# joshuagryphon/plastid

Measured on AMD Instinct MI355X. Metric: mapped_reads_per_sec, higher is better.
Workload: dtype int64; 1 GPU; C2: 100 M synthetic single-end reads, FivePrimeMapFactory(offset=12), 20 k yeast-scale transcripts; records=100000000, chains=20000, segments=21031, output_positions=33373947, tiles=5922

## Files before the change

### include/plastid_counts.h

```cpp
#ifndef PLASTID_COUNTS_H
#define PLASTID_COUNTS_H

#include <stdint.h>

#ifdef __cplusplus
extern "C" {
#endif

#define PC_ABI_VERSION 23

typedef struct pc_engine pc_engine;
typedef struct pc_plan pc_plan;

#define PC_OK 0
#define PC_ERR_ARG (-1)
#define PC_ERR_HIP (-2)
#define PC_ERR_NOMEM (-3)
#define PC_ERR_UNSORTED (-4)
#define PC_ERR_STATE (-5)

#define PC_MAP_FIVE 0
#define PC_MAP_THREE 1
#define PC_MAP_CENTER 2
#define PC_MAP_VAR5 3
#define PC_MAP_STRAT5 4

#define PC_STRAND_UNDEF 0
#define PC_STRAND_FWD 1
#define PC_STRAND_REV 2
#define PC_STRAND_UNS 3
#define PC_STRAND_NOFILTER 0x10

#define PC_FLAG_REVERSE 0x01
#define PC_FLAG_EXCLUDED 0x80

#define PC_OUT_INT64 0
#define PC_OUT_FLOAT64 1

#define PC_OFFSET_TABLE_LEN 10000
#define PC_MAX_ALIGNED_LEN 65535

const char *pc_last_error(void);
int pc_abi_version(void);
int pc_device_count(void);

int pc_create(int device, pc_engine **out);
int pc_destroy(pc_engine *e);
int pc_release_cached_memory(int device);
int pc_host_alloc(pc_engine *e, uint64_t bytes, void **out);
int pc_host_free(pc_engine *e, void *p);
int pc_reload_knobs(pc_engine *e);

int pc_clear_alignments(pc_engine *e);
int pc_add_alignment_file(pc_engine *e, int64_t n, int32_t ntid, const int32_t *tid,
                          const int32_t *pos, const uint16_t *alen, const uint8_t *flags,
                          const uint8_t *nblk, int64_t nrun, const int32_t *blk_start,
                          const int32_t *blk_len);
int pc_add_alignment_file_wide(pc_engine *e, int64_t n, int32_t ntid, const int32_t *tid,
                               const int32_t *pos, const uint16_t *alen, const uint8_t *flags,
                               const uint8_t *nblk, int64_t nrun, const int32_t *blk_start,
                               const int32_t *blk_len, int64_t n_wide, const int64_t *wide_idx,
                               const int32_t *wide_alen, const int32_t *wide_nblk);
int pc_update_flags(pc_engine *e, int file, int64_t n, const uint8_t *flags);
int pc_num_files(pc_engine *e);
int64_t pc_num_records(pc_engine *e, int file);
int64_t pc_stream_entries(pc_engine *e, int file);
int64_t pc_canonical_entries(pc_engine *e, int file);
int64_t pc_dense_cells(pc_engine *e, int file);
#define PC_DENSE_PATH_NONE 0
#define PC_DENSE_PATH_ITEMS 1
#define PC_DENSE_PATH_CHUNKS 2
int pc_dense_path(pc_engine *e);
int pc_read_records(pc_engine *e, int file, int64_t n, const int64_t *idx, int32_t *tid, int32_t *pos, int32_t *alen, uint8_t *reverse,
                    int32_t *nblk, uint16_t *flag16, uint8_t *mapq);
int pc_read_record_runs(pc_engine *e, int file, int64_t n, const int64_t *idx, const int64_t *run_at, int64_t nruns, int32_t *start,
                        int32_t *len);

int pc_set_alignment_sam(pc_engine *e, int file, int64_t n, const uint16_t *flag, const uint8_t *mapq);
int pc_set_flag_filter(pc_engine *e, int enabled, uint32_t require, uint32_t exclude, int min_mapq);
int pc_set_alignment_nh(pc_engine *e, int file, int64_t n, const uint16_t *nh);
int pc_set_nh_filter(pc_engine *e, int max_nh);

int pc_set_mapping(pc_engine *e, int kind, int param, const int32_t *fw, const int32_t *rc,
                   int table_len, int min_len, int max_len);
int pc_set_size_filter(pc_engine *e, int enabled, int min_len, int max_len);
int pc_set_normalize(pc_engine *e, int enabled, double sum);
int pc_mapping_rows(pc_engine *e);

int pc_plan_create(pc_engine *e, int64_t nseg, const int32_t *tid, const int64_t *start,
                   const int64_t *end, const uint8_t *strand, const int64_t *out_off,
                   const int8_t *out_step, const int64_t *row_stride, int64_t out_elems, int rows,
                   pc_plan **out);
int pc_plan_destroy(pc_plan *p);
int pc_plan_coordinates(pc_engine *e, pc_plan *p, int64_t *host_out, int64_t out_elems);
int64_t pc_plan_positions(pc_plan *p);
int64_t pc_plan_tiles(pc_plan *p);
int pc_plan_table(pc_plan *p, int which, void *buf, int64_t cap_bytes, int64_t *bytes);

int pc_count(pc_engine *e, pc_plan *p, int out_dtype);
int pc_sync(pc_engine *e);
int pc_query_segment(pc_engine *e, int32_t tid, int64_t start, int64_t end, uint8_t strand, int reverse_out, int out_dtype,
                     void *host_out);
int pc_read_counts(pc_engine *e, pc_plan *p, void *host_out, int64_t out_elems);
void *pc_counts_device_ptr(pc_plan *p);
void *pc_stream(pc_engine *e);

int pc_rle(pc_engine *e, pc_plan *p, int64_t period, int64_t *n_runs);
int pc_read_rle(pc_engine *e, pc_plan *p, int64_t *starts, void *values, int64_t n_runs);

int pc_warn_flags(pc_engine *e, pc_plan *p, uint8_t *flags);
int pc_warn_details(pc_engine *e, pc_plan *p, uint8_t *flags, int32_t *last_len);

int pc_total(pc_engine *e, pc_plan *p, void *host_out8);
void *pc_total_device_ptr(pc_plan *p);

int pc_mapped_reads(pc_engine *e, int file, int64_t rec_lo, int64_t rec_hi, int32_t tid,
                    int64_t start, int64_t end, uint8_t strand, uint8_t *mask);

int pc_mapped_reads_batch(pc_engine *e, pc_plan *p, int64_t *offsets, int64_t *total);
int pc_read_mapped_reads(pc_engine *e, pc_plan *p, uint32_t *rec, int64_t total);

int pc_set_profiling(pc_engine *e, int level);
int pc_last_timing(pc_engine *e, double *ms, int n);
int64_t pc_last_algorithmic_bytes(pc_engine *e);
int pc_center_replay_steps(pc_engine *e, pc_plan *p, int64_t *steps, int64_t *waves);
int pc_center_row_fill(pc_engine *e, pc_plan *p, int64_t *row_entries, int64_t *row_slots);
int pc_stream_probe(pc_engine *e, int64_t bytes, int iters, double *read_gbps, double *write_gbps);

typedef struct pc_bam pc_bam;
int pc_bam_open(pc_engine *e, const void *image, int64_t size, const char *name , pc_bam **out);
int pc_bam_counts(pc_bam *b, int64_t *counts8);
int pc_bam_timing(pc_bam *b, double *ms4);
int pc_bam_nref(pc_bam *b);
const char *pc_bam_ref_name(pc_bam *b, int i);
int32_t pc_bam_ref_length(pc_bam *b, int i);
int pc_bam_read(pc_bam *b, int32_t *tid, int32_t *pos, uint16_t *alen, uint8_t *flags, uint8_t *nblk, int32_t *blk_start,
                int32_t *blk_len, int64_t *wide_idx, int32_t *wide_alen, int32_t *wide_nblk);
int pc_bam_read_sam(pc_bam *b, uint16_t *flag, uint8_t *mapq, int32_t *lseq);
int pc_bam_read_nh(pc_bam *b, uint16_t *nh);
int pc_bam_close(pc_bam *b);
int pc_add_alignment_bam(pc_engine *e, const void *image, int64_t size, const char *name, int64_t *mapped);
int pc_bam_open_path(pc_engine *e, const char *path, pc_bam **out);
int pc_add_alignment_bam_path(pc_engine *e, const char *path, int64_t *mapped);
int pc_bam_open_span(pc_engine *e, const char *path, uint64_t voff_begin, uint64_t voff_end, int nreg, const int32_t *tid,
                     const int64_t *beg, const int64_t *end, pc_bam **out);
int pc_add_alignment_bam_span(pc_engine *e, const char *path, uint64_t voff_begin, uint64_t voff_end, int nreg, const int32_t *tid,
                              const int64_t *beg, const int64_t *end, int64_t *mapped);
int pc_bam_open_chunks(pc_engine *e, const char *path, int nchunk, const uint64_t *voff_beg, const uint64_t *voff_end, int nreg,
                       const int32_t *tid, const int64_t *beg, const int64_t *end, pc_bam **out);
int pc_add_alignment_bam_chunks(pc_engine *e, const char *path, int nchunk, const uint64_t *voff_beg, const uint64_t *voff_end,
                                int nreg, const int32_t *tid, const int64_t *beg, const int64_t *end, int64_t *mapped);
int pc_bam_stats(pc_bam *b, int64_t *out4);
#define PC_BAM_SORT 1u
int pc_bam_open_flags(pc_engine *e, const void *image, int64_t size, const char *name, uint32_t flags, pc_bam **out);
int pc_bam_open_path_flags(pc_engine *e, const char *path, uint32_t flags, pc_bam **out);
int pc_add_alignment_bam_flags(pc_engine *e, const void *image, int64_t size, const char *name, uint32_t flags, int64_t *mapped);
int pc_add_alignment_bam_path_flags(pc_engine *e, const char *path, uint32_t flags, int64_t *mapped);
int pc_bam_sort_stats(pc_bam *b, int64_t *out4, double *ms);
int pc_bam_read_file_order(pc_bam *b, int64_t *rec_no);

int pc_sam_open_path_flags(pc_engine *e, const char *path, uint32_t flags, pc_bam **out);
int pc_sam_open_flags(pc_engine *e, const void *image, int64_t size, const char *name, uint32_t flags, pc_bam **out);
int pc_add_alignment_sam_path_flags(pc_engine *e, const char *path, uint32_t flags, int64_t *mapped);

typedef struct pc_bam_index pc_bam_index;
int pc_bam_index_build(pc_engine *e, const char *path, pc_bam_index **out);
int pc_bam_index_finish(int n_ref, int64_t n_runs, const int32_t *run_tid, const uint32_t *run_bin, const uint64_t *run_beg,
                        const uint64_t *run_end, const int64_t *lin_start, const uint64_t *linear, const uint64_t *ref_beg,
                        const uint64_t *ref_end, const int64_t *ref_mapped, const int64_t *ref_unmapped, int64_t n_no_coor,
                        pc_bam_index **out);
int pc_bam_index_build_csi(pc_engine *e, const char *path, int min_shift, pc_bam_index **out);
int pc_bam_index_finish_csi(int min_shift, int n_lvls, int n_ref, int64_t n_runs, const int32_t *run_tid, const uint32_t *run_bin,
                            const uint64_t *run_beg, const uint64_t *run_end, const uint64_t *run_loff, const uint64_t *ref_beg,
                            const uint64_t *ref_end, const int64_t *ref_mapped, const int64_t *ref_unmapped, int64_t n_no_coor,
                            pc_bam_index **out);
int pc_bam_index_bytes(pc_bam_index *idx, void *buf, int64_t cap, int64_t *bytes);
int pc_bam_index_stats(pc_bam_index *idx, int64_t *out8);
int pc_bam_index_timing(pc_bam_index *idx, double *ms8);
int pc_bam_index_close(pc_bam_index *idx);

typedef struct pc_track pc_track;
int pc_track_create(pc_engine *e, int nstrands, int64_t min_chr_size, pc_track **out);
int pc_track_destroy(pc_track *t);
int pc_track_declare(pc_track *t, const char *name, int64_t length);
int pc_track_add_text(pc_track *t, const void *image, int64_t size, const char *name, int strand_slot);
int pc_track_add_path(pc_track *t, const char *path, int strand_slot);
int pc_track_num_contigs(pc_track *t);
const char *pc_track_contig_name(pc_track *t, int i);
int64_t pc_track_contig_length(pc_track *t, int i);
int64_t pc_track_contig_extent(pc_track *t, int i, int strand_slot);
int pc_track_gather(pc_track *t, int64_t nseg, const int32_t *contig, const int32_t *strand_slot, const int64_t *start, const int64_t *end,
                    const int64_t *out_off, const int8_t *out_step, int64_t out_elems, int normalize, double *host_out);
int pc_track_sum(pc_track *t, double *sum);
int pc_track_stats(pc_track *t, int64_t *out6);
int pc_track_timing(pc_track *t, double *ms5);

int pc_track_set(pc_track *t, const char *contig, int strand_slot, int64_t nseg, const int64_t *start, const int64_t *end, const int64_t *val_off,
                 const int8_t *val_step, const double *values, int64_t nvalues, double scalar);
int pc_track_combine(pc_track *a, pc_track *b, double scalar, int op, int mode_all, int64_t length_pad, int nstrands_out, const int32_t *slot_a,
                     const int32_t *slot_b, pc_track **out);
int pc_track_equal(pc_track *a, pc_track *b, int64_t npair, const int32_t *contig_a, const int32_t *slot_a, const int32_t *contig_b, const int32_t *slot_b,
                   double tol, int *equal);
int pc_track_nonzero_count(pc_track *t, int64_t *counts);
int pc_track_nonzero_read(pc_track *t, int64_t *out, int64_t total);
int pc_track_export(pc_track *t, int kind, int strand_slot, int64_t *bytes);
int pc_track_export_read(pc_track *t, void *dst, int64_t bytes);
int pc_track_export_stats(pc_track *t, int64_t *out4);
int pc_track_export_timing(pc_track *t, double *ms6);
int pc_track_export_geometry(int *out2);

int pc_counts_export_batches(int64_t n, const int64_t *len, int64_t budget, int32_t *batch_of, int *nbatch);
int pc_counts_export(pc_engine *e, pc_plan *p, int kind, int64_t period, int nrange, const char *const *names, const int64_t *elem_off,
                     const int64_t *len, int64_t *bytes);
int pc_counts_export_read(pc_engine *e, void *dst, int64_t bytes);
int pc_counts_export_stats(pc_engine *e, int64_t *out4);
int pc_counts_export_timing(pc_engine *e, double *ms6);
int pc_track_set_counts(pc_track *t, const char *contig, int strand_slot, int64_t start, pc_plan *p, int64_t elem_off, int64_t n);

int pc_bigwig_info(const char *path, const void *image, int64_t size, int64_t *out5, int max_contigs, char *names, int64_t names_bytes, int64_t *sizes);
int pc_bigwig_blocks(const char *path, const void *image, int64_t size, int64_t nblocks, int64_t *off, int64_t *bytes);
// ... 40 lines not shown
```

### plastid_amd/_lib.py

```python
import ctypes
import os

from .exceptions import EngineError

HERE = os.path.dirname(os.path.abspath(__file__))
LIB_PATH = os.environ.get("PLASTID_AMD_LIB") or os.path.join(HERE, "libplastid_counts.so")

PC_OK = 0
PC_ERR_ARG = -1
PC_ERR_HIP = -2
PC_ERR_NOMEM = -3
PC_ERR_UNSORTED = -4
PC_ERR_STATE = -5

MAP_FIVE, MAP_THREE, MAP_CENTER, MAP_VAR5, MAP_STRAT5 = 0, 1, 2, 3, 4
STRAND_UNDEF, STRAND_FWD, STRAND_REV, STRAND_UNS = 0, 1, 2, 3
STRAND_NOFILTER = 0x10
OUT_INT64, OUT_FLOAT64 = 0, 1
OFFSET_TABLE_LEN = 10000

_vp, _i64, _i32, _int = ctypes.c_void_p, ctypes.c_int64, ctypes.c_int32, ctypes.c_int
_pp = ctypes.POINTER(ctypes.c_void_p)
SIGNATURES = {
    "pc_last_error": (ctypes.c_char_p, []),
    "pc_abi_version": (_int, []),
    "pc_device_count": (_int, []),
    "pc_create": (_int, [_int, _pp]),
    "pc_destroy": (_int, [_vp]),
    "pc_reload_knobs": (_int, [_vp]),
    "pc_clear_alignments": (_int, [_vp]),
    "pc_add_alignment_file": (_int, [_vp, _i64, _i32, _vp, _vp, _vp, _vp, _vp, _i64, _vp, _vp]),
    "pc_add_alignment_file_wide": (_int, [_vp, _i64, _i32, _vp, _vp, _vp, _vp, _vp, _i64, _vp, _vp, _i64, _vp, _vp, _vp]),
    "pc_update_flags": (_int, [_vp, _int, _i64, _vp]),
    "pc_set_alignment_sam": (_int, [_vp, _int, _i64, _vp, _vp]),
    "pc_set_flag_filter": (_int, [_vp, _int, ctypes.c_uint32, ctypes.c_uint32, _int]),
    "pc_set_alignment_nh": (_int, [_vp, _int, _i64, _vp]),
    "pc_set_nh_filter": (_int, [_vp, _int]),
    "pc_num_files": (_int, [_vp]),
    "pc_num_records": (_i64, [_vp, _int]),
    "pc_stream_entries": (_i64, [_vp, _int]),
    "pc_canonical_entries": (_i64, [_vp, _int]),
    "pc_dense_cells": (_i64, [_vp, _int]),
    "pc_dense_path": (_int, [_vp]),
    "pc_read_records": (_int, [_vp, _int, _i64] + [_vp] * 8),
    "pc_read_record_runs": (_int, [_vp, _int, _i64, _vp, _vp, _i64, _vp, _vp]),
    "pc_set_mapping": (_int, [_vp, _int, _int, _vp, _vp, _int, _int, _int]),
    "pc_set_size_filter": (_int, [_vp, _int, _int, _int]),
    "pc_set_normalize": (_int, [_vp, _int, ctypes.c_double]),
    "pc_mapping_rows": (_int, [_vp]),
    "pc_plan_create": (_int, [_vp, _i64, _vp, _vp, _vp, _vp, _vp, _vp, _vp, _i64, _int, _pp]),
    "pc_plan_destroy": (_int, [_vp]),
    "pc_plan_positions": (_i64, [_vp]),
    "pc_plan_coordinates": (_int, [_vp, _vp, _vp, _i64]),
    "pc_plan_tiles": (_i64, [_vp]),
    "pc_plan_table": (_int, [_vp, _int, _vp, _i64, ctypes.POINTER(_i64)]),
    "pc_count": (_int, [_vp, _vp, _int]),
    "pc_sync": (_int, [_vp]),
    "pc_query_segment": (_int, [_vp, _i32, _i64, _i64, ctypes.c_uint8, _int, _int, _vp]),
    "pc_release_cached_memory": (_int, [_int]),
    "pc_host_alloc": (_int, [_vp, ctypes.c_uint64, ctypes.POINTER(ctypes.c_void_p)]),
    "pc_host_free": (_int, [_vp, _vp]),
    "pc_read_counts": (_int, [_vp, _vp, _vp, _i64]),
    "pc_counts_device_ptr": (_vp, [_vp]),
    "pc_stream": (_vp, [_vp]),
    "pc_rle": (_int, [_vp, _vp, _i64, ctypes.POINTER(_i64)]),
    "pc_read_rle": (_int, [_vp, _vp, _vp, _vp, _i64]),
    "pc_warn_flags": (_int, [_vp, _vp, _vp]),
    "pc_warn_details": (_int, [_vp, _vp, _vp, _vp]),
    "pc_total": (_int, [_vp, _vp, _vp]),
    "pc_total_device_ptr": (_vp, [_vp]),
    "pc_mapped_reads": (_int, [_vp, _int, _i64, _i64, _i32, _i64, _i64, ctypes.c_uint8, _vp]),
    "pc_mapped_reads_batch": (_int, [_vp, _vp, _vp, ctypes.POINTER(_i64)]),
    "pc_read_mapped_reads": (_int, [_vp, _vp, _vp, _i64]),
    "pc_set_profiling": (_int, [_vp, _int]),
    "pc_last_timing": (_int, [_vp, _vp, _int]),
    "pc_last_algorithmic_bytes": (_i64, [_vp]),
    "pc_center_replay_steps": (_int, [_vp, _vp, ctypes.POINTER(_i64), ctypes.POINTER(_i64)]),
    "pc_center_row_fill": (_int, [_vp, _vp, ctypes.POINTER(_i64), ctypes.POINTER(_i64)]),
    "pc_stream_probe": (_int, [_vp, _i64, _int, _vp, _vp]),
    "pc_bam_open": (_int, [_vp, _vp, _i64, ctypes.c_char_p, _pp]),
    "pc_bam_counts": (_int, [_vp, _vp]),
    "pc_bam_timing": (_int, [_vp, _vp]),
    "pc_bam_nref": (_int, [_vp]),
    "pc_bam_ref_name": (ctypes.c_char_p, [_vp, _int]),
    "pc_bam_ref_length": (_i32, [_vp, _int]),
    "pc_bam_read": (_int, [_vp] * 11),
    "pc_bam_read_sam": (_int, [_vp, _vp, _vp, _vp]),
    "pc_bam_read_nh": (_int, [_vp, _vp]),
    "pc_bam_close": (_int, [_vp]),
    "pc_add_alignment_bam": (_int, [_vp, _vp, _i64, ctypes.c_char_p, ctypes.POINTER(_i64)]),
    "pc_bam_open_path": (_int, [_vp, ctypes.c_char_p, _pp]),
    "pc_add_alignment_bam_path": (_int, [_vp, ctypes.c_char_p, ctypes.POINTER(_i64)]),
    "pc_bam_open_span": (_int, [_vp, ctypes.c_char_p, ctypes.c_uint64, ctypes.c_uint64, _int, _vp, _vp, _vp, _pp]),
    "pc_add_alignment_bam_span": (_int, [_vp, ctypes.c_char_p, ctypes.c_uint64, ctypes.c_uint64, _int, _vp, _vp, _vp, ctypes.POINTER(_i64)]),
    "pc_bam_open_chunks": (_int, [_vp, ctypes.c_char_p, _int, _vp, _vp, _int, _vp, _vp, _vp, _pp]),
    "pc_add_alignment_bam_chunks": (_int, [_vp, ctypes.c_char_p, _int, _vp, _vp, _int, _vp, _vp, _vp, ctypes.POINTER(_i64)]),
    "pc_bam_stats": (_int, [_vp, _vp]),
    "pc_bam_open_flags": (_int, [_vp, _vp, _i64, ctypes.c_char_p, ctypes.c_uint32, _pp]),
    "pc_bam_open_path_flags": (_int, [_vp, ctypes.c_char_p, ctypes.c_uint32, _pp]),
    "pc_add_alignment_bam_flags": (_int, [_vp, _vp, _i64, ctypes.c_char_p, ctypes.c_uint32, ctypes.POINTER(_i64)]),
    "pc_add_alignment_bam_path_flags": (_int, [_vp, ctypes.c_char_p, ctypes.c_uint32, ctypes.POINTER(_i64)]),
    "pc_bam_sort_stats": (_int, [_vp, _vp, _vp]),
    "pc_bam_read_file_order": (_int, [_vp, _vp]),
    "pc_sam_open_path_flags": (_int, [_vp, ctypes.c_char_p, ctypes.c_uint32, _pp]),
    "pc_sam_open_flags": (_int, [_vp, _vp, _i64, ctypes.c_char_p, ctypes.c_uint32, _pp]),
    "pc_add_alignment_sam_path_flags": (_int, [_vp, ctypes.c_char_p, ctypes.c_uint32, ctypes.POINTER(_i64)]),
    "pc_bam_index_build": (_int, [_vp, ctypes.c_char_p, _pp]),
    "pc_bam_index_finish": (_int, [_int, _i64] + [_vp] * 10 + [_i64, _pp]),
    "pc_bam_index_build_csi": (_int, [_vp, ctypes.c_char_p, _int, _pp]),
    "pc_bam_index_finish_csi": (_int, [_int, _int, _int, _i64] + [_vp] * 9 + [_i64, _pp]),
    "pc_bam_index_bytes": (_int, [_vp, _vp, _i64, ctypes.POINTER(_i64)]),
    "pc_bam_index_stats": (_int, [_vp, _vp]),
    "pc_bam_index_timing": (_int, [_vp, _vp]),
    "pc_bam_index_close": (_int, [_vp]),
    "pc_track_create": (_int, [_vp, _int, _i64, _pp]),
    "pc_track_destroy": (_int, [_vp]),
    "pc_track_declare": (_int, [_vp, ctypes.c_char_p, _i64]),
    "pc_track_add_text": (_int, [_vp, _vp, _i64, ctypes.c_char_p, _int]),
    "pc_track_add_path": (_int, [_vp, ctypes.c_char_p, _int]),
    "pc_track_num_contigs": (_int, [_vp]),
    "pc_track_contig_name": (ctypes.c_char_p, [_vp, _int]),
    "pc_track_contig_length": (_i64, [_vp, _int]),
    "pc_track_contig_extent": (_i64, [_vp, _int, _int]),
    "pc_track_gather": (_int, [_vp, _i64, _vp, _vp, _vp, _vp, _vp, _vp, _i64, _int, _vp]),
    "pc_track_sum": (_int, [_vp, ctypes.POINTER(ctypes.c_double)]),
    "pc_track_stats": (_int, [_vp, _vp]),
    "pc_track_timing": (_int, [_vp, _vp]),
    "pc_track_set": (_int, [_vp, ctypes.c_char_p, _int, _i64, _vp, _vp, _vp, _vp, _vp, _i64, ctypes.c_double]),
    "pc_track_combine": (_int, [_vp, _vp, ctypes.c_double, _int, _int, _i64, _int, _vp, _vp, _pp]),
    "pc_track_equal": (_int, [_vp, _vp, _i64, _vp, _vp, _vp, _vp, ctypes.c_double, ctypes.POINTER(_int)]),
    "pc_track_nonzero_count": (_int, [_vp, _vp]),
    "pc_track_nonzero_read": (_int, [_vp, _vp, _i64]),
    "pc_track_export": (_int, [_vp, _int, _int, ctypes.POINTER(_i64)]),
    "pc_track_export_read": (_int, [_vp, _vp, _i64]),
    "pc_track_export_stats": (_int, [_vp, _vp]),
    "pc_track_export_timing": (_int, [_vp, _vp]),
    "pc_track_export_geometry": (_int, [_vp]),
    "pc_counts_export_batches": (_int, [_i64, _vp, _i64, _vp, ctypes.POINTER(_int)]),
    "pc_counts_export": (_int, [_vp, _vp, _int, _i64, _int, _vp, _vp, _vp, ctypes.POINTER(_i64)]),
    "pc_counts_export_read": (_int, [_vp, _vp, _i64]),
    "pc_counts_export_stats": (_int, [_vp, _vp]),
    "pc_counts_export_timing": (_int, [_vp, _vp]),
    "pc_track_set_counts": (_int, [_vp, ctypes.c_char_p, _int, _i64, _vp, _i64, _i64]),
    "pc_bigwig_info": (_int, [ctypes.c_char_p, _vp, _i64, _vp, _int, _vp, _i64, _vp]),
    "pc_bigwig_blocks": (_int, [ctypes.c_char_p, _vp, _i64, _i64, _vp, _vp]),
    "pc_inflate_zlib": (_int, [_vp, _vp, _i64, _vp, _vp, _i64, _vp, _vp, _vp]),
    "pc_deflate_zlib": (_int, [_vp, _vp, _i64, _vp, _vp, _vp, _i64, _vp, _vp]),
    "pc_deflate_zlib_mode": (_int, [_vp, _vp, _i64, _vp, _vp, _vp, _i64, _vp, _vp, _int]),
    "pc_huffman_lengths": (_int, [_vp, _vp, _i64, _int, _vp]),
    "pc_track_export_bigwig": (_int, [_vp, _int, _i64, _i64, _int, _vp]),
    "pc_track_export_bigwig_zoom": (_int, [_vp, _int, _i64, _i64, _int, _i64, _vp]),
    "pc_track_export_bigwig_read": (_int, [_vp, _vp, _i64]),
    "pc_track_set_length": (_int, [_vp, ctypes.c_char_p, _i64]),
    "pc_track_bigwig_export_stats": (_int, [_vp, _vp]),
    "pc_track_bigwig_export_block_types": (_int, [_vp, _vp]),
    "pc_track_bigwig_export_timing": (_int, [_vp, _vp]),
    "pc_track_bigwig_export_zoom_stats": (_int, [_vp, _vp, _vp]),
    "pc_track_bigwig_export_zoom_timing": (_int, [_vp, _vp]),
    "pc_track_add_bigwig": (_int, [_vp, _vp, _i64, ctypes.c_char_p, _int]),
    "pc_track_add_bigwig_path": (_int, [_vp, ctypes.c_char_p, _int]),
    "pc_track_bigwig_stats": (_int, [_vp, _vp]),
    "pc_track_bigwig_timing": (_int, [_vp, _vp]),
    "pc_track_gather_sum": (_int, [_int, _vp, _i64, _vp, _vp, _vp, _vp, _vp, _vp, _i64, _int, ctypes.c_double, _vp]),
    "pc_track_sum_ranges": (_int, [_vp, _i64, _vp, _vp, _vp, _vp, ctypes.POINTER(ctypes.c_double)]),
    "pc_bigwig_summary_open": (_int, [_vp, _vp, _i64, ctypes.c_char_p, _pp]),
    "pc_bigwig_summary_open_path": (_int, [_vp, ctypes.c_char_p, _pp]),
    "pc_bigwig_summary_close": (_int, [_vp]),
    "pc_bigwig_summary_query": (_int, [_vp, _i64, _vp, _vp, _vp, _i64, _vp]),
    "pc_bigwig_summary_stats": (_int, [_vp, _vp, _int, _vp]),
    "pc_bigwig_summary_timing": (_int, [_vp, _vp]),
}

_lib = None


PC_BAM_SORT = 1

ABI_VERSION = 23


def load():
    global _lib
    if _lib is not None:
        return _lib
    if not os.path.exists(LIB_PATH):
        raise EngineError(
            "HIP counting library %s is missing. Build it with "
            "`python -m plastid_amd.build` (needs hipcc, gfx950). "
            "There is no CPU fallback." % LIB_PATH)
    try:
        lib = ctypes.CDLL(LIB_PATH)
    except OSError as e:
        raise EngineError("cannot load %s: %s" % (LIB_PATH, e))
    try:
        lib.pc_abi_version.restype = _int
        have = lib.pc_abi_version()
    except AttributeError:
        have = None
    if have != ABI_VERSION:
        raise EngineError("%s implements ABI revision %s, this package needs %d: rebuild it with `python -m plastid_amd.build --force`"
                          % (LIB_PATH, have, ABI_VERSION))
    for name, (res, args) in SIGNATURES.items():
        fn = getattr(lib, name)
        fn.restype = res
        fn.argtypes = args
    _lib = lib
    return lib


def last_error():
    msg = load().pc_last_error()
    return msg.decode("utf-8", "replace") if msg else ""


def check(rc, what=""):
    if rc == PC_OK:
        return
    msg = last_error() or what
    if rc in (PC_ERR_ARG, PC_ERR_UNSORTED):
        raise ValueError(msg)
    if rc == PC_ERR_NOMEM:
        raise MemoryError(msg)
    raise EngineError(msg)
```

### plastid_amd/csrc/dense_host.h

```cpp
#pragma once
#include <cstdint>

#if defined(__HIPCC__)
#define PCDENSE_HD __host__ __device__
#else
#define PCDENSE_HD
#endif

namespace pcdense {

constexpr int kItemLen = 2048;
constexpr uint32_t kEscape = 65535u;
constexpr int64_t kBytesPerCell = 2;
constexpr int64_t kBuildBlockCap = (int64_t)1 << 30;

PCDENSE_HD inline int64_t extent(int64_t declared, int64_t furthest_end) {
    const int64_t d = declared > 0 ? declared : 0, f = furthest_end > 0 ? furthest_end : 0;
    return d > f ? d : f;
}

inline int64_t layout(int ntid, const int64_t *ext, int64_t *cell_off) {
    int64_t at = 0;
    for (int t = 0; t < ntid; ++t)
        for (int s = 0; s < 2; ++s) { cell_off[2 * t + s] = at; at += ext[t]; }
    cell_off[2 * ntid] = at;
    return at;
}

struct PlanIn {
    int nfiles = 0;
    bool point_rule = false;
    int rows = 1;
    uint32_t modes = 0;
    bool has_sums = false;
    bool forbidden = false;
    int64_t cells = 0;
    int64_t stream_entries = 0;
};

inline bool plan_conditions(const PlanIn &p) {
    return !p.forbidden && p.nfiles == 1 && p.point_rule && p.rows == 1 && (p.modes & ~3u) == 0u && p.modes != 0u && !p.has_sums;
}
inline bool size_rule(int64_t cells, int64_t stream_entries) { return cells > 0 && cells * kBytesPerCell <= stream_entries * 4; }
inline bool build_fits(int64_t cells) { return cells * 8 <= kBuildBlockCap; }
inline bool eligible(const PlanIn &p) { return plan_conditions(p) && size_rule(p.cells, p.stream_entries) && build_fits(p.cells); }

struct SegIn {
    int64_t out_off = 0;
    int64_t len = 0;
    int64_t clip_lo = 0, clip_hi = 0;
    int64_t start = 0;
    int32_t step = 1;
    bool known = false;
    int64_t cell_base = 0;
    int64_t ext = 0;
};

struct Item {
    int64_t out_off;
    int64_t cell0;
    int32_t len, step, lo, hi;
};
static_assert(sizeof(Item) == 32, "Item is 32 bytes in HBM");

PCDENSE_HD inline int64_t items_of(int64_t len) { return len > 0 ? (len + kItemLen - 1) / kItemLen : 0; }

PCDENSE_HD inline Item cut_item(const SegIn &s, int64_t k) {
    const int64_t a = k * kItemLen;
    const int64_t n = s.len - a < kItemLen ? s.len - a : kItemLen;
    Item it;
    it.out_off = s.out_off + (int64_t)s.step * a;
    it.len = (int32_t)n; it.step = s.step; it.lo = 0; it.hi = 0; it.cell0 = -1;
    if (!s.known) return it;
    int64_t lo = s.clip_lo, hi = s.clip_hi;
    if (s.start + hi > s.ext) hi = s.ext - s.start;
    if (s.start + lo < 0) lo = -s.start;
    lo -= a; hi -= a;
    if (lo < 0) lo = 0;
    if (hi > n) hi = n;
    if (hi <= lo) return it;
    it.lo = (int32_t)lo; it.hi = (int32_t)hi;
    it.cell0 = s.cell_base + s.start + a;
    return it;
}

struct PairCut {
    int32_t head, pairs, tail;
};
PCDENSE_HD inline PairCut pair_cut(int64_t out_off, int32_t step, int32_t len) {
    PairCut c;
    c.head = (int32_t)((step > 0 ? out_off : out_off + 1) & 1);
    if (c.head > len) c.head = len;
    c.pairs = (len - c.head) >> 1;
    c.tail = (len - c.head) & 1;
    return c;
}
PCDENSE_HD inline int64_t pair_slot(int64_t out_off, int32_t step, const PairCut &c, int32_t p) {
    const int64_t i0 = c.head + 2 * (int64_t)p;
    return step > 0 ? out_off + i0 : out_off - i0 - 1;
}

#ifndef PC_DENSE_BATCH
#define PC_DENSE_BATCH 1
#endif
constexpr int kBatch = PC_DENSE_BATCH;
PCDENSE_HD inline int64_t batches_of(int64_t n_items) { return (n_items + kBatch - 1) / kBatch; }

#ifndef PC_DENSE_CHUNK
#define PC_DENSE_CHUNK 1024
#endif
constexpr int kChunk = PC_DENSE_CHUNK;
constexpr int kRow = 128;
constexpr int kInlineSpans = 7;
static_assert(kChunk % (4 * kRow) == 0 && kChunk / kRow <= 32, "a chunk is whole rows for four waves; its rows are the bits of a word");

struct Span {
    uint32_t ab, rr;
    uint32_t cell;
    int32_t dir;
    PCDENSE_HD uint32_t a() const { return ab & 0xffffu; }
    PCDENSE_HD uint32_t b() const { return ab >> 16; }
    PCDENSE_HD uint32_t ra() const { return rr & 0xffffu; }
    PCDENSE_HD uint32_t rb() const { return rr >> 16; }
};
static_assert(sizeof(Span) == 16, "Span is 16 bytes in HBM");
struct ChunkDesc {
    uint32_t n, ovf, pad[2];
    Span s[kInlineSpans];
};
static_assert(sizeof(ChunkDesc) == 128, "a descriptor is one line");

PCDENSE_HD inline int64_t chunks_of(int64_t out_elems) { return (out_elems + kChunk - 1) / kChunk; }
PCDENSE_HD inline int64_t seg_out_lo(int64_t out_off, int32_t step, int64_t len) { return step > 0 ? out_off : out_off - len + 1; }
PCDENSE_HD inline int64_t spans_of(int64_t out_lo, int64_t len) { return len > 0 ? (out_lo + len - 1) / kChunk - out_lo / kChunk + 1 : 0; }
inline bool spans_fit(int64_t nseg, int64_t covered) { return 2 * nseg + covered / kChunk < (int64_t)0xffffffffu; }

PCDENSE_HD inline Span cut_span(const SegIn &s, int64_t k) {
    const int64_t lo = seg_out_lo(s.out_off, s.step, s.len), base = (lo / kChunk + k) * kChunk;
    const int64_t a = lo > base ? lo : base, b = lo + s.len < base + kChunk ? lo + s.len : base + kChunk;
    int64_t plo = 0, phi = 0;
    if (s.known) {
        plo = s.clip_lo; phi = s.clip_hi;
        if (s.start + phi > s.ext) phi = s.ext - s.start;
        if (s.start + plo < 0) plo = -s.start;
        if (plo < 0) plo = 0;
        if (phi > s.len) phi = s.len;
    }
    int64_t ra = s.step > 0 ? s.out_off + plo : s.out_off - phi + 1, rb = s.step > 0 ? s.out_off + phi : s.out_off - plo + 1;
    if (ra < a) ra = a;
    if (rb > b) rb = b;
    if (phi <= plo || rb <= ra) ra = rb = a;
    Span sp;
    sp.ab = (uint32_t)(a - base) | (uint32_t)(b - base) << 16;
    sp.rr = (uint32_t)(ra - base) | (uint32_t)(rb - base) << 16;
    sp.dir = s.step > 0 ? 1 : -1;
    const int64_t pos = s.step > 0 ? a - s.out_off : s.out_off - a;
    sp.cell = (uint32_t)(s.cell_base + s.start + pos);
    return sp;
}
PCDENSE_HD inline bool span_reads(const Span &s, uint32_t e) { return e >= s.ra() && e < s.rb(); }
PCDENSE_HD inline uint32_t span_cell(const Span &s, uint32_t e) { return s.cell + (uint32_t)s.dir * (e - s.a()); }
PCDENSE_HD inline uint32_t span_rows(const Span &s) {
    const uint32_t ra = s.ra(), rb = s.rb();
    return ra < rb ? (2u << ((rb - 1u) / kRow)) - (1u << (ra / kRow)) : 0u;
}
PCDENSE_HD inline uint32_t span_base(const Span &s) { return s.cell - (uint32_t)s.dir * s.a(); }
PCDENSE_HD inline uint32_t base_cell(uint32_t base, bool up, uint32_t e) { return up ? base + e : base - e; }
PCDENSE_HD inline bool same_word(uint32_t x0, uint32_t x1) { return (x0 | 1u) == (x1 | 1u); }

PCDENSE_HD inline bool out_overlap(int64_t prev_lo, int64_t prev_len, int64_t lo) { return prev_lo + prev_len > lo; }
PCDENSE_HD inline bool first_of_chunk(int64_t lo, int64_t k, int64_t prev_end) {
    return k > 0 || lo % kChunk == 0 || prev_end < 0 || (prev_end - 1) / kChunk < lo / kChunk;
}
PCDENSE_HD inline ChunkDesc make_desc(const Span *spans, uint32_t first, uint32_t n) {
    ChunkDesc d;
    d.n = n; d.ovf = first + kInlineSpans; d.pad[0] = d.pad[1] = 0;
    for (int i = 0; i < kInlineSpans; ++i) {
        if ((uint32_t)i < n) d.s[i] = spans[first + i];
        else { d.s[i].ab = d.s[i].rr = 0; d.s[i].cell = 0; d.s[i].dir = 1; }
    }
    return d;
}

}
```

### plastid_amd/csrc/plastid_counts.hip

```cpp
#include "pc_kernels.hip.h"
#include "plan_kernels.hip.h"
#include "stage_kernels.hip.h"
#include "dense_kernels.hip.h"

#include <hipcub/hipcub.hpp>

#include <algorithm>
#include <atomic>
#include <cstdarg>
#include <cstdio>
#include <cstdlib>
#include <cstring>
#include <string>
#include <chrono>
#include <future>
#include <functional>
#include <condition_variable>
#include <map>
#include <mutex>
#include <unistd.h>
#include <mutex>
#include <sched.h>
#include <sys/mman.h>
#include <sys/stat.h>
// ... 228 lines not shown
            if (hipGetDevice(&dev_now) == hipSuccess) BigReservoir::get().free_all(dev_now);
            HIP_TRY(hipMalloc((void **)&p, n * sizeof(T)));
        }
        cap = n;
        return PC_OK;
    }
    int upload(const T *src, size_t n, hipStream_t s) {
        PC_TRY(reserve(n));
        if (n) HIP_TRY(hipMemcpyAsync(p, src, n * sizeof(T), hipMemcpyHostToDevice, s));
        return PC_OK;
    }
    int upload(const std::vector<T> &v, hipStream_t s) { return upload(v.data(), v.size(), s); }
    void swap(DevBuf &o) {
        std::swap(p, o.p); std::swap(cap, o.cap); std::swap(pool, o.pool); std::swap(pool_class, o.pool_class); std::swap(big_bytes, o.big_bytes);
    }
};

struct PinnedBuf {
    uint8_t *p = nullptr;
    size_t cap = 0;
    ~PinnedBuf() { if (p) (void)hipHostFree(p); }
    int reserve(size_t n) {
        if (n <= cap) return PC_OK;
        if (p) (void)hipHostFree(p);
        p = nullptr; cap = 0;
        const size_t want = std::max<size_t>(n + n / 2, 512 * 1024);
        HIP_TRY(hipHostMalloc((void **)&p, want, hipHostMallocDefault));
        cap = want;
        return PC_OK;
    }
};

template <typename T> struct DevView {
    T *p = nullptr;
};

struct TransferJob { void *dst; const void *src; size_t bytes; };
struct TransferRing {
    static constexpr int kSlots = 12, kThreadsUp = 6, kThreadsDown = 10;
    static constexpr size_t kPiece = (size_t)16 << 20;
    uint8_t *slot[kSlots] = {};
    hipEvent_t ev[kSlots] = {};
    hipStream_t stream = nullptr;
    std::mutex busy;
    static TransferRing &of(int device) {
        static std::mutex m;
        static std::map<int, TransferRing *> *rings = new std::map<int, TransferRing *>;
        std::lock_guard<std::mutex> g(m);
        TransferRing *&r = (*rings)[device];
        if (!r) r = new TransferRing;
        return *r;
    }
    int run(int device, const std::vector<TransferJob> &jobs, size_t piece, bool always, bool down = false) {
        std::lock_guard<std::mutex> one(busy);
        HIP_TRY(hipSetDevice(device));
        if (!stream) HIP_TRY(hipStreamCreateWithFlags(&stream, hipStreamNonBlocking));
        size_t total = 0;
        for (const auto &j : jobs) total += j.bytes;
        if (total == 0) return PC_OK;
        const hipMemcpyKind kind = down ? hipMemcpyDeviceToHost : hipMemcpyHostToDevice;
        if (total < 4 * kPiece && !always) {
            for (const auto &j : jobs)
                if (j.bytes) HIP_TRY(hipMemcpyAsync(j.dst, j.src, j.bytes, kind, stream));
            HIP_TRY(hipStreamSynchronize(stream));
            return PC_OK;
        }
        piece = std::max<size_t>(1, std::min(piece, kPiece));
        std::vector<TransferJob> pieces;
        for (const auto &j : jobs) {
            if (j.bytes == 0) continue;
            hipPointerAttribute_t attr;
            const void *host_side = down ? j.dst : j.src;
            if (!always && hipPointerGetAttributes(&attr, host_side) == hipSuccess && attr.type == hipMemoryTypeHost) {
                HIP_TRY(hipMemcpyAsync(j.dst, j.src, j.bytes, kind, stream));
                continue;
            }
            (void)hipGetLastError();
            for (size_t off = 0; off < j.bytes; off += piece)
                pieces.push_back({(uint8_t *)j.dst + off, (const uint8_t *)j.src + off, std::min(piece, j.bytes - off)});
        }
        const size_t np = pieces.size();
        for (int k = 0; k < kSlots && np > 0; ++k) {
            if (!slot[k]) HIP_TRY(hipHostMalloc((void **)&slot[k], kPiece, hipHostMallocDefault));
            if (!ev[k]) HIP_TRY(hipEventCreateWithFlags(&ev[k], hipEventDisableTiming));
        }
        std::unique_ptr<std::atomic<uint8_t>[]> done(new std::atomic<uint8_t>[np]);
        for (size_t k = 0; k < np; ++k) done[k].store(0, std::memory_order_relaxed);
        std::atomic<size_t> next{0};
        std::atomic<int> failed{0};
        std::mutex order;
        auto work = [&]() {
            if (hipSetDevice(device) != hipSuccess) failed.store(1);
            for (;;) {
                const size_t p = next.fetch_add(1);
                if (p >= np) return;
                const int k = (int)(p % kSlots);
                if (p >= (size_t)kSlots) {
                    while (!done[p - kSlots].load(std::memory_order_acquire)) std::this_thread::yield();
                    if (!down && !failed.load() && hipEventSynchronize(ev[k]) != hipSuccess) failed.store(1);
                }
                if (!failed.load()) {
                    if (!down) std::memcpy(slot[k], pieces[p].src, pieces[p].bytes);
                    {
                        std::lock_guard<std::mutex> lk(order);
                        if (hipMemcpyAsync(down ? (void *)slot[k] : pieces[p].dst, down ? pieces[p].src : (const void *)slot[k], pieces[p].bytes, kind, stream) != hipSuccess ||
                            hipEventRecord(ev[k], stream) != hipSuccess)
                            failed.store(1);
                    }
                    if (down && !failed.load()) {
                        if (hipEventSynchronize(ev[k]) != hipSuccess) failed.store(1);
                        else std::memcpy(pieces[p].dst, slot[k], pieces[p].bytes);
                    }
                }
                done[p].store(1, std::memory_order_release);
            }
        };
        int T = down ? kThreadsDown : kThreadsUp;
        if (const char *env = getenv("PC_STAGE_UPLOAD_THREADS")) T = std::max(1, std::min(kSlots - 1, atoi(env)));
        T = (int)std::min<size_t>((size_t)T, np);
        std::vector<std::thread> th;
        for (int t = 1; t < T; ++t) th.emplace_back(work);
        if (np > 0) work();
        for (auto &x : th) x.join();
        const hipError_t he = hipStreamSynchronize(stream);
        if (failed.load() || he != hipSuccess) { (void)hipGetLastError(); return fail(PC_ERR_HIP, "transfer ring: a copy failed"); }
        return PC_OK;
    }
};

static int stage_threads(int64_t n) {
    int t = std::min(usable_cpus(), 32);
    if (const char *env = getenv("PC_STAGE_THREADS")) t = std::max(1, atoi(env));
    return (int)std::max<int64_t>(1, std::min<int64_t>(t, n / (1 << 20) + 1));
}

struct FilterState {
    bool ff_on = false;
    uint32_t require = 0, exclude = 0, min_mapq = 0, max_nh = 0;
    bool operator==(const FilterState &o) const {
        return ff_on == o.ff_on && require == o.require && exclude == o.exclude && min_mapq == o.min_mapq && max_nh == o.max_nh;
    }
};

struct CanonSig {
    int kind = -1, param = 0, filt_on = 0, filt_min = 0, filt_max = -1, fast_lo = 0, fast_hi = 0, Ws = 0;
    uint64_t words_gen = 0;
    std::vector<int32_t> fw, rc;
    bool operator==(const CanonSig &o) const {
        return kind == o.kind && param == o.param && filt_on == o.filt_on && filt_min == o.filt_min && filt_max == o.filt_max &&
               fast_lo == o.fast_lo && fast_hi == o.fast_hi && Ws == o.Ws && words_gen == o.words_gen && fw == o.fw && rc == o.rc;
    }
};

struct DenseSig {
    int kind = -1, param = 0, filt_on = 0, filt_min = 0, filt_max = -1;
    uint64_t words_gen = 0;
    FilterState applied;
    std::vector<int32_t> fw, rc;
    bool operator==(const DenseSig &o) const {
        return kind == o.kind && param == o.param && filt_on == o.filt_on && filt_min == o.filt_min && filt_max == o.filt_max &&
               words_gen == o.words_gen && applied == o.applied && fw == o.fw && rc == o.rc;
    }
};

struct StagedFile {
    int64_t n = 0, nrun = 0, nlong = 0;
    int W = 1;
    int64_t max_span = 1;
    DevBuf<uint2> rec;
    DevBuf<uint32_t> blk_off;
    DevBuf<int2> blk;
    DevBuf<int64_t> tid_bounds;
    DevBuf<uint32_t> long_idx;
    DevBuf<int32_t> long_tid;
    DevBuf<int32_t> long_pmax;
    DevBuf<int64_t> long_tid_bounds;
    DevBuf<uint4> long_rec;
    int64_t ngap = 0;
    DevBuf<uint4> gap_rec;
    DevBuf<int4> gap_runs, long_runs;
    DevBuf<int64_t> gap_tid_bounds;
    DevBuf<uint32_t> lin_tab, glin_tab, llin_tab, plin_tab;
    DevBuf<int64_t> lin_off;
    std::vector<int64_t> len_hist;
    int len_min = 65536, len_max = -1;
    int slen_min = 0, slen_max = 0;
    int tlen_min = 0, tlen_max = 0;
    DevBuf<uint32_t> stream;
    DevBuf<uint32_t> cstream, clin_tab;
    int64_t cn = -1;
    uint64_t words_gen = 0;
    DevBuf<uint32_t> kstream, klin_tab;
    DevBuf<int16_t> kshift;
    int64_t kn = -1;
    bool ksig_valid = false;
    CanonSig ksig;
    uint64_t kid = 0;
    std::vector<int64_t> tid_end;
    std::vector<int64_t> dext, dcell_off;
    int64_t dcells = -1;
    DevBuf<int64_t> d_dext, d_dcell_off;
    DevBuf<uint16_t> dense;
    DevBuf<uint32_t> dovf_key, dovf_val;
    uint32_t dn_ovf = 0;
    bool dsig_valid = false;
    DenseSig dsig;
    uint64_t did = 0;
    size_t nlin = 0;
    int64_t nrunrec = 0;
    int Wr = 1;
    DevBuf<uint2> run_rec;
    DevBuf<uint32_t> run_recidx;
    DevBuf<uint32_t> rlin_tab;
    int64_t nxlong = 0;
    int Wg = 1;
    DevBuf<uint4> xlong_rec;
    DevBuf<int4> xlong_runs;
    DevBuf<uint32_t> xllin_tab, xplin_tab;
    int64_t nwide = 0;
    DevBuf<uint2> long_wide, xlong_wide, wide_val;
    DevBuf<uint32_t> wide_rec;
    DevBuf<uint16_t> sam_flag;
    DevBuf<uint8_t> sam_mapq;
    bool have_sam = false;
    DevBuf<uint16_t> sam_nh;
    bool have_nh = false;
    FilterState applied;
    bool applied_valid = true;
    DevBuf<uint2> cs_ent[3];
    DevBuf<uint32_t> cs_soff[3];
    int64_t cs_n[3] = {-1, -1, -1};
    int cs_nib[3] = {-1, -1, -1};
    FileView view() const {
        FileView v;
        v.rec = rec.p; v.blk_off = blk_off.p; v.blk = blk.p; v.tid_bounds = tid_bounds.p;
        v.stream = stream.p;
        v.cstream = cn >= 0 ? cstream.p : nullptr; v.clin_tab = cn >= 0 ? clin_tab.p : nullptr;
        v.long_idx = long_idx.p; v.long_tid = long_tid.p; v.long_pmax = long_pmax.p;
        v.long_tid_bounds = long_tid_bounds.p; v.long_rec = long_rec.p; v.n = n; v.nlong = nlong;
        v.gap_rec = gap_rec.p; v.gap_tid_bounds = gap_tid_bounds.p; v.ngap = ngap;
        v.gap_runs = gap_runs.p; v.long_runs = long_runs.p;
        v.lin_tab = lin_tab.p; v.glin_tab = glin_tab.p; v.llin_tab = llin_tab.p; v.plin_tab = plin_tab.p; v.lin_off = lin_off.p;
        v.run_rec = run_rec.p; v.rlin_tab = rlin_tab.p; v.nrunrec = nrunrec;
        v.xlong_rec = xlong_rec.p; v.xlong_runs = xlong_runs.p; v.xllin_tab = xllin_tab.p; v.xplin_tab = xplin_tab.p; v.nxlong = nxlong;
        for (int k = 0; k < 3; ++k) {
            v.cs_ent[k] = cs_n[k] >= 0 ? cs_ent[k].p : nullptr; v.cs_soff[k] = cs_n[k] >= 0 ? cs_soff[k].p : nullptr;
            v.cs_total[k] = cs_n[k] >= 0 ? (uint32_t)cs_n[k] : 0u;
            v.cs_indirect[k] = len_max > 255 ? 1u : 0u;
        }
        v.long_wide = nwide ? long_wide.p : nullptr; v.xlong_wide = nwide ? xlong_wide.p : nullptr;
        v.wide_rec = wide_rec.p; v.wide_val = wide_val.p; v.nwide = nwide;
        return v;
    }
};

}

struct Knobs {
    int tile_g = 0;
    int64_t work_r = 49152;
    int64_t pile = 0;
    int no_small = 0;
    int small_rows = 0;
    int64_t ranges_cg16_max = (int64_t)1 << 19;
    int ranges_cg1 = 0;
    int64_t first_sync_spare = 65536;
    int hist_memset = 0;
    int64_t hist_lazy_bytes = (int64_t)64 << 20;
    int no_stream_probe = 0;
    int no_compact = 0;
    double compact_keep = 0.9;
    int no_canon = 0;
    int no_dense = 0;
    int dense_items = 0;
    int dense_debug = 0;
    int no_single = 0;
    int plan_build = 0;
    int small_g = 512;
    int64_t small_n = 8192;
    int debug_work = 0;
    int test_stale_counts = 0;
    int center_t1 = 8;
    int center_t2 = 4;
    int64_t center_floor = 32768;
    int center_lds = 0;
    int center_per_wave = 0;
    int center_debug = 0;
    void load() {
        *this = Knobs();
        if (const char *env = getenv("PC_TILE_G")) tile_g = std::max(256, atoi(env) / 256 * 256);
        if (const char *env = getenv("PC_WORK_R")) work_r = std::max(1024, atoi(env));
        if (const char *env = getenv("PC_PILE")) pile = std::max<int64_t>(work_r, atoll(env));
        no_small = getenv("PC_NO_SMALL") ? 1 : 0;
        if (const char *env = getenv("PC_SMALL_ROWS")) small_rows = atoi(env);
        no_single = getenv("PC_NO_SINGLE") ? 1 : 0;
        no_compact = getenv("PC_NO_COMPACT") ? 1 : 0;
        no_canon = getenv("PC_NO_CANON") ? 1 : 0;
        no_dense = getenv("PC_NO_DENSE") ? 1 : 0;
        dense_items = getenv("PC_DENSE_ITEMS") ? 1 : 0;
        dense_debug = getenv("PC_DENSE_DEBUG") ? 1 : 0;
        if (const char *env = getenv("PC_COMPACT_KEEP")) compact_keep = std::min(1.0, std::max(0.0, atof(env)));
        no_stream_probe = getenv("PC_NO_STREAM_PROBE") ? 1 : 0;
        hist_memset = getenv("PC_HIST_MEMSET") ? 1 : 0;
        hist_lazy_bytes = getenv("PC_HIST_LAZY_BYTES") ? std::max<int64_t>(1, atoll(getenv("PC_HIST_LAZY_BYTES"))) : ((int64_t)64 << 20);
        ranges_cg1 = getenv("PC_RANGES_CG1") ? 1 : 0;
        ranges_cg16_max = getenv("PC_RANGES_CG16_MAX") ? atoll(getenv("PC_RANGES_CG16_MAX")) : ((int64_t)1 << 19);
        first_sync_spare = getenv("PC_FIRST_SYNC_SPARE") ? atoll(getenv("PC_FIRST_SYNC_SPARE")) : 65536;
        if (const char *env = getenv("PC_PLAN_BUILD")) plan_build = std::strcmp(env, "host") == 0 ? 1 : (std::strcmp(env, "gpu") == 0 ? 2 : 0);
        if (const char *env = getenv("PC_SMALL_G")) small_g = std::max(64, atoi(env) / 64 * 64);
        if (const char *env = getenv("PC_SMALL_N")) small_n = std::max(64, atoi(env));
        debug_work = getenv("PC_DEBUG_WORK") ? 1 : 0;
        test_stale_counts = getenv("PC_TEST_STALE_COUNTS") ? 1 : 0;
        if (const char *env = getenv("PC_CENTER_T1")) center_t1 = std::max(8, atoi(env));
        if (const char *env = getenv("PC_CENTER_T2")) center_t2 = std::max(1, atoi(env));
        if (const char *env = getenv("PC_CENTER_FLOOR")) center_floor = std::max(64, atoi(env));
        center_debug = getenv("PC_CENTER_DEBUG") ? 1 : 0;
        if (const char *env = getenv("PC_CENTER_LDS")) center_lds = std::max(0, atoi(env));
    }
};

static void destroy_tracks_of(pc_engine *e);
static void destroy_summaries_of(pc_engine *e);

struct pc_engine {
    DevPool pool;
    DevBuf<uint8_t> plan_scratch[3];
    Knobs knobs;
    int device = 0;
    hipStream_t stream = nullptr;
    hipStream_t side_stream = nullptr;
    static constexpr int kAux = 3;
    hipStream_t aux_stream[kAux] = {nullptr, nullptr, nullptr};
    hipEvent_t ev_fork = nullptr, ev_join = nullptr;
    std::vector<hipStream_t> parked_streams;
    hipEvent_t ev_pinned = nullptr;
    hipEvent_t ev[8] = {};
    std::vector<StagedFile *> files;
    std::vector<pc_track *> tracks;
    std::vector<pc_bigwig_summary *> summaries;
    DevBuf<uint8_t> cx_text;
    int64_t cx_bytes = -1;
    int64_t cx_stats[4] = {0, 0, 0, 0};
    double cx_ms[6] = {0, 0, 0, 0, 0, 0};
    int ntid = 0;
    DevBuf<FileView> d_files;
    bool files_dirty = true;
    bool have_map = false;
    int kind = PC_MAP_CENTER, param = 0, min_len = 25, max_len = 35, rows = 1, table_len = 0;
    std::vector<int32_t> h_fw, h_rc;
    DevBuf<int32_t> d_fw, d_rc;
    int filt_on = 0, filt_min = 0, filt_max = -1;
    int norm_on = 0;
    double norm_sum = 1.0;
    DevBuf<double> d_inv;
    DevBuf<double> d_invh;
    DevBuf<double> d_cvalh;
    DevBuf<uint32_t> d_counters;
    DevBuf<uint8_t> d_flags;
    uint8_t *q_host = nullptr;
    void *q_dev = nullptr;
    uint32_t q_seq = 0;
    bool ff_on = false;
    uint32_t ff_require = 0, ff_exclude = 0, ff_min_mapq = 0;
    uint32_t ff_max_nh = 0;
    bool filter_on() const { return ff_on || ff_max_nh != 0u; }
    FilterState filter_state() const {
        FilterState s;
        s.ff_on = ff_on; s.require = ff_require; s.exclude = ff_exclude; s.min_mapq = ff_min_mapq; s.max_nh = ff_max_nh;
        return s;
    }
    bool pinned_busy = false;
    PinnedBuf pinned;
    PinnedBuf bam_ring[2];
    hipEvent_t ev_ring[2] = {nullptr, nullptr};
    uint64_t work_generation = 1;
    size_t max_lds = 64 * 1024;
    DevBuf<double> d_partial;
    DevBuf<Unmappable> d_unmap;
    double last_ms[6] = {0, 0, 0, 0, 0, 0};
    bool timing_valid = false;
    int prof_level = 0;
    int timed_level = 0;
    int64_t last_alg_bytes = 0;
    bool last_count_dense = false;
    int last_dense_path = PC_DENSE_PATH_NONE;
    bool want_center_steps = false;
    int64_t center_steps = 0, center_waves = 0;

    MapParams params() const {
        MapParams mp;
        mp.kind = kind; mp.param = param; mp.min_len = min_len; mp.max_len = max_len; mp.rows = rows;
        mp.filt_on = filt_on; mp.filt_min = filt_min; mp.filt_max = filt_max;
        mp.table_len = table_len; mp.fw = d_fw.p; mp.rc = d_rc.p;
        return mp;
    }
    int max_over_files(int StagedFile::*field) const {
        int w = 1;
        for (auto *f : files) w = std::max(w, f->*field);
        return w;
    }
    int W() const { return max_over_files(&StagedFile::W); }
    int Wg() const { return max_over_files(&StagedFile::Wg); }
    int Wr() const { return max_over_files(&StagedFile::Wr); }
    int Ws() const { return max_over_files(&StagedFile::slen_max); }
};

struct pc_plan {
    pc_engine *e = nullptr;
    int64_t nseg = 0, out_elems = 0, covered = 0;
    int rows = 1, G = 4096;
    uint32_t modes = 0;
    int max_slots = 1;
    int64_t npos = 0;
    HostPlan host;
    size_t n_tiles = 0, n_pieces = 0, n_opieces = 0;
    size_t n_cchunks = 0, n_gchunks = 0;
    bool gpu_built = false;
    bool host_inputs = true;
    DevBuf<uint8_t> d_inputs;
    DevBuf<GatherSeg> d_gsegs_own;
    bool has_sums = false;
    bool out_needs_zero = false;
    bool no_dense = false;
    DevBuf<pcdense::Item> d_ditems;
    uint32_t n_ditems = 0;
    uint64_t ditems_id = 0;
    DevBuf<pcdense::ChunkDesc> d_dchunks;
    DevBuf<pcdense::Span> d_dspans;
    bool chunks_ok = false;
    uint64_t dchunks_id = 0;
    bool hist_clean = false;
    bool hist_lazy = false;
    bool center_ready = false, gather_ready = false;
    DevBuf<uint8_t> d_tables2, d_tables3;
    std::vector<int32_t> h_tid;
    std::vector<int64_t> h_start, h_end;
    std::vector<uint8_t> h_strand;
    DevBuf<uint8_t> d_tables;
    DevView<Tile> d_tiles;
    DevView<Piece> d_pieces;
    DevView<OutPiece> d_opieces;
    DevView<CenterChunk> d_cchunks;
    DevBuf<uint32_t> d_corder;
    DevBuf<uint32_t> d_ccand;
    DevBuf<uint32_t> d_rle_cnt;
    DevBuf<int64_t> d_rle_base;
    DevBuf<int64_t> d_rle_starts;
    DevBuf<unsigned long long> d_rle_values;
    int64_t rle_runs = -1;
    DevBuf<u32x4> d_cranges;
    DevBuf<u32x2> d_crec;
    DevBuf<uint32_t> d_crows;
    DevBuf<uint32_t> d_ccounts;
    DevBuf<CenterSlot> d_cslots;
    uint64_t center_generation = 0;
    int center_W = -1;
    int center_nfiles = 0;
    uint32_t *h_center_counts = nullptr;
    hipEvent_t ev_center_counts = nullptr;
    bool center_counts_known = false;
    uint32_t center_counts[2] = {0, 0};
    DevView<GatherSeg> d_gsegs;
    DevView<GatherChunk> d_gchunks;
    DevView<uint32_t> d_tile_items;
    bool tile_items_zero = false;
    struct WorkKey {
        uint64_t generation = 0;
        int nfiles = 0, G = 0, Wg = 0, Ws = 0, Wr = 0, small_g = 0;
        int64_t R = 0, pile = 0, small_n = 0, cap = 0;
        uint64_t canon = 0;
        bool operator==(const WorkKey &o) const {
            return canon == o.canon && generation == o.generation && nfiles == o.nfiles && G == o.G && Wg == o.Wg && Ws == o.Ws && Wr == o.Wr &&
                   small_g == o.small_g && R == o.R && pile == o.pile && small_n == o.small_n && cap == o.cap;
        }
    };
    WorkKey work_key;
    bool work_valid = false;
    DevBuf<WorkItem> d_work, d_work_small;
    DevBuf<FileRange> d_chain, d_chain_small;
    DevView<uint32_t> d_wcounters;
    bool wcounters_zero = false;
    DevView<uint8_t> d_hist;
    DevBuf<uint8_t> d_hist_own;
    DevBuf<uint8_t> d_out;
    DevBuf<unsigned long long> d_mr_off;
    DevBuf<uint32_t> d_mr_rec;
    int64_t mr_total = -1;
    DevView<uint8_t> d_total;
    int last_dtype = -1;
    bool counted = false;
// ... 384 lines not shown
    p->gather_ready = true;
    return PC_OK;
}

int build_center_stream(pc_engine *e, StagedFile *sf, int sel, int nib) {
    hipStream_t st = e->stream;
    const int64_t n = sf->n;
    if (sf->cs_n[sel] >= 0 && sf->cs_nib[sel] == nib) return PC_OK;
    if (n + sf->nrun >= (int64_t)0xffffffffu)
        return fail(PC_ERR_ARG, "pc_count: the center rule takes at most 2^32-2 aligned runs per file (%lld records, %lld runs of multi-run reads); split the file",
                    (long long)n, (long long)sf->nrun);
    if (sf->cs_n[sel] < 0) {
        PC_TRY(sf->cs_soff[sel].reserve((size_t)n + 1));
        hipLaunchKernelGGL(k_cs_count, dim3((unsigned)((n + 1 + kWG - 1) / kWG)), dim3(kWG), 0, st, sf->rec.p, n, sel, sf->cs_soff[sel].p);
        {
            size_t tmp_bytes = 0;
            DevBuf<uint8_t> d_tmp;
            HIP_TRY(hipcub::DeviceScan::ExclusiveSum(nullptr, tmp_bytes, sf->cs_soff[sel].p, sf->cs_soff[sel].p, (int)(n + 1), st));
            PC_TRY(d_tmp.reserve(tmp_bytes));
            HIP_TRY(hipcub::DeviceScan::ExclusiveSum(d_tmp.p, tmp_bytes, sf->cs_soff[sel].p, sf->cs_soff[sel].p, (int)(n + 1), st));
            HIP_TRY(hipStreamSynchronize(st));
        }
        uint32_t total = 0;
        HIP_TRY(hipMemcpy(&total, sf->cs_soff[sel].p + n, sizeof(total), hipMemcpyDeviceToHost));
        PC_TRY(sf->cs_ent[sel].reserve((size_t)total + 64));
        sf->cs_n[sel] = (int64_t)total;
        e->files_dirty = true;
    }
    hipLaunchKernelGGL(k_cs_scatter, dim3((unsigned)((n + 64 + kWG - 1) / kWG)), dim3(kWG), 0, st, sf->rec.p, sf->blk_off.p, sf->blk.p, n,
                       sel, nib, sf->cs_soff[sel].p, sf->cs_ent[sel].p);
    HIP_TRY(hipGetLastError());
    sf->cs_nib[sel] = nib;
    return PC_OK;
}


}

namespace {
__global__ void k_stream_probe_wait(uint32_t *flag, unsigned long long budget) {
    const unsigned long long t0 = wall_clock64();
    uint32_t seen = 0;
    while ((seen = __hip_atomic_load(flag, __ATOMIC_RELAXED, __HIP_MEMORY_SCOPE_AGENT)) == 0u && wall_clock64() - t0 < budget)
        __builtin_amdgcn_s_sleep(16);
    flag[1] = seen;
}
__global__ void k_stream_probe_set(uint32_t *flag) { __hip_atomic_store(flag, 1u, __ATOMIC_RELAXED, __HIP_MEMORY_SCOPE_AGENT); }

int streams_run_side_by_side(pc_engine *e, hipStream_t a, hipStream_t b, uint32_t *flag) {
    HIP_TRY(hipMemsetAsync(flag, 0, 2 * sizeof(uint32_t), a));
    HIP_TRY(hipEventRecord(e->ev_fork, a));
    HIP_TRY(hipStreamWaitEvent(b, e->ev_fork, 0));
    hipLaunchKernelGGL(k_stream_probe_wait, dim3(1), dim3(1), 0, a, flag, 50000ull);
    hipLaunchKernelGGL(k_stream_probe_set, dim3(1), dim3(1), 0, b, flag);
    HIP_TRY(hipGetLastError());
    HIP_TRY(hipStreamSynchronize(a));
    HIP_TRY(hipStreamSynchronize(b));
    uint32_t seen[2] = {0, 0};
    HIP_TRY(hipMemcpy(seen, flag, sizeof(seen), hipMemcpyDeviceToHost));
    return seen[1] ? 1 : 0;
}

int settle_streams(pc_engine *e) {
    if (e->knobs.no_stream_probe) return PC_OK;
    DevBuf<uint32_t> flag;
    flag.pool = &e->pool;
    PC_TRY(flag.reserve(2));
    auto settle = [&](hipStream_t &cand, std::initializer_list<hipStream_t> beside) -> int {
        for (int attempt = 0;; ++attempt) {
            int ok = 1;
            for (hipStream_t other : beside) {
                ok = streams_run_side_by_side(e, other, cand, flag.p);
                if (ok <= 0) break;
            }
            if (ok < 0) return ok;
            if (ok || attempt == 7) return PC_OK;
            hipStream_t fresh = nullptr;
            HIP_TRY(hipStreamCreateWithFlags(&fresh, hipStreamNonBlocking));
            e->parked_streams.push_back(cand);
            cand = fresh;
        }
    };
    int rc = settle(e->side_stream, {e->stream});
    if (rc == PC_OK) rc = settle(e->aux_stream[0], {e->stream, e->side_stream});
    return rc;
}
}

extern "C" {

const char *pc_last_error(void) { return g_err.c_str(); }
int pc_abi_version(void) { return PC_ABI_VERSION; }

int pc_device_count(void) {
    int n = 0;
    if (hipGetDeviceCount(&n) != hipSuccess) return 0;
    return n;
}

int pc_create(int device, pc_engine **out) {
    if (!out) return fail(PC_ERR_ARG, "pc_create: out is NULL");
    *out = nullptr;
    int ndev = 0;
    hipError_t err = hipGetDeviceCount(&ndev);
    if (err != hipSuccess || ndev <= 0)
        return fail(PC_ERR_HIP, "pc_create: no HIP device available (%s); this engine has no CPU fallback",
                    err == hipSuccess ? "device count is 0" : hipGetErrorString(err));
    if (device < 0 || device >= ndev) return fail(PC_ERR_ARG, "pc_create: device %d out of range [0,%d)", device, ndev);
    HIP_TRY(hipSetDevice(device));
    pc_engine *e = new pc_engine();
    e->device = device;
    e->pool.device = device;
    e->knobs.load();
    BigReservoir::get().engine_created(device);
    HIP_TRY(hipStreamCreateWithFlags(&e->stream, hipStreamNonBlocking));
    HIP_TRY(hipStreamCreateWithFlags(&e->side_stream, hipStreamNonBlocking));
    for (auto &a : e->aux_stream) HIP_TRY(hipStreamCreateWithFlags(&a, hipStreamNonBlocking));
    HIP_TRY(hipEventCreateWithFlags(&e->ev_fork, hipEventDisableTiming));
    HIP_TRY(hipEventCreateWithFlags(&e->ev_pinned, hipEventDisableTiming));
    HIP_TRY(hipEventCreateWithFlags(&e->ev_join, hipEventDisableTiming));
    {
        int lds_attr = 0;
        if (hipDeviceGetAttribute(&lds_attr, hipDeviceAttributeMaxSharedMemoryPerBlock, device) == hipSuccess && lds_attr > 0)
            e->max_lds = (size_t)lds_attr;
    }
    for (auto &ev : e->ev) HIP_TRY(hipEventCreate(&ev));
    std::vector<double> inv(65536);
    inv[0] = 0.0;
    for (int m = 1; m < 65536; ++m) inv[m] = 1.0 / (double)m;
    int rc = e->d_inv.upload(inv, e->stream);
    std::vector<double> invh(65536);
    for (int m = 0; m < 65536; ++m) invh[m] = inv[m] * 0.5;
    if (rc == PC_OK) rc = e->d_invh.upload(invh, e->stream);
    if (rc == PC_OK) rc = e->d_counters.reserve(16);
    if (rc == PC_OK && hipMemsetAsync(e->d_counters.p, 0, 16 * sizeof(uint32_t), e->stream) != hipSuccess) rc = fail(PC_ERR_HIP, "pc_create: memset failed");
    if (rc == PC_OK && hipStreamSynchronize(e->stream) != hipSuccess) rc = fail(PC_ERR_HIP, "pc_create: sync failed");
    if (rc == PC_OK) rc = settle_streams(e);
    if (rc != PC_OK) {
        pc_destroy(e);
        return rc;
    }
    *out = e;
    return PC_OK;
}

int pc_destroy(pc_engine *e) {
    if (!e) return PC_OK;
    (void)hipSetDevice(e->device);
    if (e->stream) (void)hipStreamSynchronize(e->stream);
    destroy_tracks_of(e);
    destroy_summaries_of(e);
    for (auto *f : e->files) delete f;
    e->files.clear();
    for (auto &ev : e->ev)
        if (ev) (void)hipEventDestroy(ev);
    if (e->side_stream) { (void)hipStreamSynchronize(e->side_stream); (void)hipStreamDestroy(e->side_stream); }
    for (auto &a : e->aux_stream) if (a) { (void)hipStreamSynchronize(a); (void)hipStreamDestroy(a); }
    for (auto a : e->parked_streams) if (a) (void)hipStreamDestroy(a);
    if (e->q_host) (void)hipHostFree(e->q_host);
    if (e->ev_fork) (void)hipEventDestroy(e->ev_fork);
    if (e->ev_pinned) (void)hipEventDestroy(e->ev_pinned);
    for (auto &x : e->ev_ring) if (x) (void)hipEventDestroy(x);
    if (e->ev_join) (void)hipEventDestroy(e->ev_join);
    if (e->stream) (void)hipStreamDestroy(e->stream);
    const int device = e->device;
    delete e;
    BigReservoir::get().engine_destroyed(device);
    return PC_OK;
}

int pc_release_cached_memory(int device) {
    int ndev = 0;
    if (hipGetDeviceCount(&ndev) != hipSuccess || device < 0 || device >= ndev) return fail(PC_ERR_ARG, "pc_release_cached_memory: device %d out of range", device);
    HIP_TRY(hipSetDevice(device));
    BigReservoir::get().free_all(device);
    return PC_OK;
}

int pc_host_alloc(pc_engine *e, uint64_t bytes, void **out) {
    if (!e || !out) return fail(PC_ERR_ARG, "pc_host_alloc: engine / out is NULL");
    *out = nullptr;
    HIP_TRY(hipSetDevice(e->device));
    void *p = nullptr;
    HIP_TRY(hipHostMalloc(&p, std::max<uint64_t>(bytes, 8), hipHostMallocDefault));
    *out = p;
    return PC_OK;
}

int pc_host_free(pc_engine *e, void *p) {
    if (!e) return fail(PC_ERR_ARG, "pc_host_free: engine is NULL");
    if (!p) return PC_OK;
    HIP_TRY(hipSetDevice(e->device));
    HIP_TRY(hipStreamSynchronize(e->stream));
    HIP_TRY(hipHostFree(p));
    return PC_OK;
}

int pc_reload_knobs(pc_engine *e) {
    if (!e) return fail(PC_ERR_ARG, "engine is NULL");
    e->knobs.load();
    e->work_generation += 1;
    return PC_OK;
}

int pc_clear_alignments(pc_engine *e) {
    if (!e) return fail(PC_ERR_ARG, "engine is NULL");
    HIP_TRY(hipSetDevice(e->device));
    HIP_TRY(hipStreamSynchronize(e->stream));
    for (auto *f : e->files) delete f;
    e->files.clear();
    e->ntid = 0;
    e->files_dirty = true;
    e->work_generation += 1;
    return PC_OK;
}

int pc_num_files(pc_engine *e) { return e ? (int)e->files.size() : 0; }
int64_t pc_num_records(pc_engine *e, int file) {
    if (!e || file < 0 || file >= (int)e->files.size()) return -1;
    return e->files[file]->n;
}
int64_t pc_stream_entries(pc_engine *e, int file) {
    if (!e || file < 0 || file >= (int)e->files.size()) return -1;
    const StagedFile *sf = e->files[file];
    return sf->cn >= 0 ? sf->cn : sf->n;
}
int64_t pc_canonical_entries(pc_engine *e, int file) {
    if (!e || file < 0 || file >= (int)e->files.size()) return -1;
    const StagedFile *sf = e->files[file];
    if (e->files.size() != 1) return -1;
    return (!e->knobs.no_canon && sf->ksig_valid && sf->ksig.words_gen == sf->words_gen) ? sf->kn : -1;
}

namespace {
}

int pc_read_records(pc_engine *e, int file, int64_t n, const int64_t *idx, int32_t *tid, int32_t *pos, int32_t *alen, uint8_t *reverse,
                    int32_t *nblk, uint16_t *flag16, uint8_t *mapq) {
    if (!e || file < 0 || file >= (int)e->files.size()) return fail(PC_ERR_ARG, "pc_read_records: bad file index");
    if (n < 0 || (n > 0 && (!idx || !tid || !pos || !alen || !reverse || !nblk))) return fail(PC_ERR_ARG, "pc_read_records: bad arguments");
    if (n == 0) return PC_OK;
    StagedFile *sf = e->files[file];
    for (int64_t k = 0; k < n; ++k)
        if (idx[k] < 0 || idx[k] >= sf->n) return fail(PC_ERR_ARG, "pc_read_records: record index %lld out of range", (long long)idx[k]);
    HIP_TRY(hipSetDevice(e->device));
    PoolScope pool_scope(&e->pool);
    hipStream_t st = e->stream;
    DevBuf<int64_t> d_idx;
    DevBuf<uint8_t> d_out;
    int rc = d_idx.upload(idx, (size_t)n, st);
    if (rc == PC_OK) rc = d_out.reserve((size_t)n * 20 + 64);
    if (rc != PC_OK) return rc;
    int32_t *o_tid = (int32_t *)d_out.p, *o_pos = o_tid + n, *o_alen = o_pos + n, *o_nblk = o_alen + n;
    uint16_t *o_f16 = (uint16_t *)(o_nblk + n);
    uint8_t *o_rev = (uint8_t *)(o_f16 + n), *o_mq = o_rev + n;
    hipLaunchKernelGGL(k_gather_records, dim3((unsigned)((n + kWG - 1) / kWG)), dim3(kWG), 0, st, sf->view(), e->ntid, d_idx.p, n,
                       sf->have_sam ? sf->sam_flag.p : nullptr, sf->have_sam ? sf->sam_mapq.p : nullptr, o_tid, o_pos, o_alen, o_rev, o_nblk, o_f16, o_mq);
    HIP_TRY(hipGetLastError());
    HIP_TRY(hipMemcpyAsync(tid, o_tid, (size_t)n * 4, hipMemcpyDeviceToHost, st));
    HIP_TRY(hipMemcpyAsync(pos, o_pos, (size_t)n * 4, hipMemcpyDeviceToHost, st));
    HIP_TRY(hipMemcpyAsync(alen, o_alen, (size_t)n * 4, hipMemcpyDeviceToHost, st));
    HIP_TRY(hipMemcpyAsync(nblk, o_nblk, (size_t)n * 4, hipMemcpyDeviceToHost, st));
    HIP_TRY(hipMemcpyAsync(reverse, o_rev, (size_t)n, hipMemcpyDeviceToHost, st));
    if (flag16) HIP_TRY(hipMemcpyAsync(flag16, o_f16, (size_t)n * 2, hipMemcpyDeviceToHost, st));
    if (mapq) HIP_TRY(hipMemcpyAsync(mapq, o_mq, (size_t)n, hipMemcpyDeviceToHost, st));
    HIP_TRY(hipStreamSynchronize(st));
    return PC_OK;
}

int pc_read_record_runs(pc_engine *e, int file, int64_t n, const int64_t *idx, const int64_t *run_at, int64_t nruns, int32_t *start, int32_t *len) {
    if (!e || file < 0 || file >= (int)e->files.size()) return fail(PC_ERR_ARG, "pc_read_record_runs: bad file index");
    if (n < 0 || nruns < 0 || (n > 0 && (!idx || !run_at)) || (nruns > 0 && (!start || !len))) return fail(PC_ERR_ARG, "pc_read_record_runs: bad arguments");
    if (n == 0 || nruns == 0) return PC_OK;
    StagedFile *sf = e->files[file];
    for (int64_t k = 0; k < n; ++k) {
        if (idx[k] < 0 || idx[k] >= sf->n) return fail(PC_ERR_ARG, "pc_read_record_runs: record index %lld out of range", (long long)idx[k]);
        if (run_at[k] < 0 || run_at[k] > nruns || (k > 0 && run_at[k] < run_at[k - 1])) return fail(PC_ERR_ARG, "pc_read_record_runs: run offsets must ascend within [0, nruns]");
    }
    HIP_TRY(hipSetDevice(e->device));
    PoolScope pool_scope(&e->pool);
    hipStream_t st = e->stream;
    DevBuf<int64_t> d_idx, d_at;
    DevBuf<int32_t> d_runs;
    int rc = d_idx.upload(idx, (size_t)n, st);
    if (rc == PC_OK) rc = d_at.upload(run_at, (size_t)n, st);
    if (rc == PC_OK) rc = d_runs.reserve((size_t)nruns * 2);
    if (rc != PC_OK) return rc;
    hipLaunchKernelGGL(k_gather_runs, dim3((unsigned)((n + kWG - 1) / kWG)), dim3(kWG), 0, st, sf->view(), d_idx.p, n, d_at.p, d_runs.p, d_runs.p + nruns);
    HIP_TRY(hipGetLastError());
    HIP_TRY(hipMemcpyAsync(start, d_runs.p, (size_t)nruns * 4, hipMemcpyDeviceToHost, st));
    HIP_TRY(hipMemcpyAsync(len, d_runs.p + nruns, (size_t)nruns * 4, hipMemcpyDeviceToHost, st));
    HIP_TRY(hipStreamSynchronize(st));
    return PC_OK;
}

int pc_add_alignment_file(pc_engine *e, int64_t n, int32_t ntid, const int32_t *tid, const int32_t *pos,
                          const uint16_t *alen, const uint8_t *flags, const uint8_t *nblk, int64_t nrun,
                          const int32_t *blk_start, const int32_t *blk_len) {
    return pc_add_alignment_file_wide(e, n, ntid, tid, pos, alen, flags, nblk, nrun, blk_start, blk_len, 0, nullptr, nullptr, nullptr);
}

static int build_compact_stream(pc_engine *e, StagedFile *sf, int ntid);

}

namespace {

struct StageInput {
    int64_t n = 0;
    int32_t ntid = 0;
    const int32_t *tid = nullptr, *pos = nullptr;
    const uint16_t *alen = nullptr;
    const uint8_t *flags = nullptr, *nblk = nullptr;
    int64_t nrun = 0;
    const int32_t *blk_start = nullptr, *blk_len = nullptr;
    int64_t n_wide = 0;
    const int64_t *wide_idx = nullptr;
    const int32_t *wide_alen = nullptr, *wide_nblk = nullptr;
    const pcstage::DevCols *dev = nullptr;
};

struct FileStats {
    std::vector<int64_t> span_hist, gap_span_hist, wide_span_hist, len_hist, len1_hist, tid_end;
    std::vector<int32_t> last_pos;
    int Wr = 1, rmin = 65536, rmax = -1;
    int64_t max_span = 1;
    explicit FileStats(int ntid)
        : span_hist(pcstage::kSpanBins, 0), gap_span_hist(pcstage::kSpanBins, 0), wide_span_hist(pcstage::kSpanBins, 0), len_hist(pcstage::kLenBins, 0),
          len1_hist(pcstage::kLen1Bins, 0), tid_end((size_t)ntid, 0), last_pos((size_t)ntid, -1) {}
};

struct StageCall {
    const StageInput &in;
    StageClock clk;
    DevBuf<int32_t> d_pos, d_bs, d_bl;
    DevBuf<uint16_t> d_alen;
    DevBuf<uint8_t> d_flags8, d_nblk8;
    pcstage::DevCols cols;
    std::vector<int64_t> tid_bounds;
    int64_t n_ok;
    DevBuf<uint32_t> d_run_at;
    int64_t nrunrec = 0;
    DevBuf<uint2> d_val_in;
    DevBuf<uint32_t> d_idx_in;
    FileStats stats;
    int wcap = 64;
    uint32_t nwg = 0;
    DevBuf<uint32_t> d_side_at;
    size_t side_total[3] = {0, 0, 0};
    std::vector<int64_t> lin_off;
    explicit StageCall(const StageInput &i) : in(i), cols(), tid_bounds((size_t)i.ntid + 1, 0), n_ok(i.n), stats(i.ntid) {}
};

int finish_phase(hipStream_t st, hipError_t he, const char *what) {
    if (he == hipSuccess) he = hipGetLastError();
    const hipError_t waited = hipStreamSynchronize(st);
    if (he == hipSuccess) he = waited;
    return he == hipSuccess ? PC_OK : fail(PC_ERR_HIP, what, hipGetErrorString(he));
}

template <class... Bufs> int reserve_all(size_t n, Bufs &...bufs) {
    int rc = PC_OK;
    (void)(((rc = bufs.reserve(n)) == PC_OK) && ...);
// ... 696 lines not shown
    p->nseg = nseg;
    p->out_elems = out_elems;
    p->rows = rows;
    int rc;
    if (on_gpu) rc = plan_build_gpu(e, p, nseg, tid, start, end, strand, out_off, out_step, row_stride, out_elems, rows);
    else {
        p->G = hp.G; p->modes = hp.modes; p->max_slots = hp.max_slots; p->npos = hp.npos;
        p->covered = hp.covered; p->has_sums = hp.has_sums; p->out_needs_zero = hp.out_needs_zero;
        p->host = std::move(hp);
        p->h_tid.assign(tid, tid + nseg);
        p->h_start.assign(start, start + nseg);
        p->h_end.assign(end, end + nseg);
        p->h_strand.assign(strand, strand + nseg);
        rc = plan_upload(e, p);
    }
    if (rc != PC_OK) {
        (void)hipStreamSynchronize(e->stream);
        delete p;
        return rc;
    }
    *out = p;
    return PC_OK;
}

int pc_plan_destroy(pc_plan *p) {
    if (!p) return PC_OK;
    if (p->e) {
        (void)hipSetDevice(p->e->device);
        (void)hipStreamSynchronize(p->e->stream);
    }
    delete p;
    return PC_OK;
}

int64_t pc_plan_positions(pc_plan *p) { return p ? p->npos : -1; }
int64_t pc_plan_tiles(pc_plan *p) { return p ? (int64_t)p->n_tiles : -1; }

int pc_plan_table(pc_plan *p, int which, void *buf, int64_t cap_bytes, int64_t *bytes) {
    if (!p || !bytes || which < 0 || which > 4 || cap_bytes < 0 || (cap_bytes > 0 && !buf)) return fail(PC_ERR_ARG, "pc_plan_table: bad arguments");
    HIP_TRY(hipSetDevice(p->e->device));
    HIP_TRY(hipStreamSynchronize(p->e->stream));
    if (which == 4) {
        const int64_t v[12] = {p->G, (int64_t)p->modes, p->max_slots, p->npos, p->covered, p->has_sums ? 1 : 0, p->out_needs_zero ? 1 : 0,
                               (int64_t)p->n_tiles, (int64_t)p->n_pieces, (int64_t)p->n_opieces, p->gpu_built ? 1 : 0, p->nseg};
        *bytes = (int64_t)sizeof(v);
        std::memcpy(buf, v, (size_t)std::min<int64_t>(cap_bytes, *bytes));
        return PC_OK;
    }
    const void *src = nullptr;
    size_t n = 0;
    bool on_host = false;
    if (which == 0) { src = p->d_tiles.p; n = p->n_tiles * sizeof(Tile); }
    else if (which == 1) { src = p->d_pieces.p; n = p->n_pieces * sizeof(Piece); }
    else if (which == 2) { src = p->d_opieces.p; n = p->n_opieces * sizeof(OutPiece); }
    else if (p->gpu_built) { src = p->d_gsegs_own.p; n = (size_t)p->nseg * sizeof(GatherSeg); }
    else { src = p->host.gsegs.data(); n = p->host.gsegs.size() * sizeof(GatherSeg); on_host = true; }
    *bytes = (int64_t)n;
    const size_t take = (size_t)std::min<int64_t>(cap_bytes, (int64_t)n);
    if (take) {
        if (on_host) std::memcpy(buf, src, take);
        else HIP_TRY(hipMemcpy(buf, src, take, hipMemcpyDeviceToHost));
    }
    return PC_OK;
}

}

namespace {

template <int... Vs, class F>
void dispatch_int(int v, F &&launch) {
    (void)((v == Vs ? (launch(std::integral_constant<int, Vs>{}), true) : false) || ...);
}

template <bool STRAT, class F>
void dispatch_hist(int kind, int outmode, F &&launch) {
    const int k = kind == PC_MAP_FIVE ? 0 : kind == PC_MAP_THREE ? 1 : (STRAT && kind == PC_MAP_STRAT5) ? 4 : 3;
    dispatch_int<0, 1, 2>(outmode, [&](auto O) {
        if constexpr (STRAT) dispatch_int<0, 1, 3, 4>(k, [&](auto K) { launch(K, O); });
        else dispatch_int<0, 1, 3>(k, [&](auto K) { launch(K, O); });
    });
}

struct HistLds {
    int tab_lo = 0, tab_n = 0, fast_lo = 0, fast_hi = 0;
    size_t table_words = 0;
};

HistLds hist_lds_shape(const pc_engine *e) {
    HistLds s;
    int lmin = 65536, lmax = -1;
    s.fast_lo = kStreamMaxLen;
    for (auto *f : e->files) {
        lmin = std::min(lmin, f->len_min); lmax = std::max(lmax, f->len_max);
        s.fast_lo = std::min(s.fast_lo, f->tlen_min); s.fast_hi = std::max(s.fast_hi, f->tlen_max);
    }
    if ((e->kind == PC_MAP_VAR5 || e->kind == PC_MAP_STRAT5) && lmax >= lmin) {
        s.tab_lo = lmin;
        s.tab_n = std::max(0, std::min(std::min(lmax, e->table_len - 1) - lmin + 1, 1024));
    }
    s.fast_lo = std::min(s.fast_lo, s.fast_hi);
    const size_t stage_words = (size_t)kOpStage * sizeof(OutPiece) / sizeof(uint32_t);
    s.table_words = (size_t)((s.tab_n + 3) & ~3) + stage_words + (size_t)(s.fast_hi + 1) * kModes + 64;
    return s;
}

struct CountCall {
    int out_dtype;
    int outmode;
    int nfiles, ntiles;
    int64_t nrec, nextra;
    size_t hist_bytes;
    MapParams mp;
};

int mark(pc_engine *e, int k) {
    if (e->prof_level >= ((k == 1 || k == 4) ? 2 : 1)) HIP_TRY(hipEventRecord(e->ev[k], e->stream));
    return PC_OK;
}

int count_validate(pc_engine *e, pc_plan *p, int out_dtype) {
    if (!e || !p || p->e != e) return fail(PC_ERR_ARG, "pc_count: bad engine/plan");
    if (!e->have_map) return fail(PC_ERR_STATE, "pc_count: no mapping rule set (pc_set_mapping)");
    if (e->files.empty()) return fail(PC_ERR_STATE, "pc_count: no alignments staged (pc_add_alignment_file)");
    if (out_dtype != PC_OUT_INT64 && out_dtype != PC_OUT_FLOAT64) return fail(PC_ERR_ARG, "pc_count: bad out_dtype");
    if (p->rows != e->rows) return fail(PC_ERR_ARG, "pc_count: plan built for %d rows, mapping rule has %d", p->rows, e->rows);
    PC_TRY(check_filter_columns(e, "pc_count"));
    const bool float_only = e->kind == PC_MAP_CENTER || e->norm_on;
    if (float_only && out_dtype != PC_OUT_FLOAT64)
        return fail(PC_ERR_ARG, "pc_count: center mapping / normalisation produce float64 (map_factories.pyx:230, genome_array.py:826-827)");
    if (p->has_sums && float_only)
        return fail(PC_ERR_ARG, "pc_count: summed slices (out_step 0) need an integer mapping rule without normalisation");
    return PC_OK;
}

int count_prepare(pc_engine *e, pc_plan *p, bool dense) {
    const bool center = e->kind == PC_MAP_CENTER;
    if (center) {
        PC_TRY(ensure_center_tables(e, p));
        const bool need[3] = {(p->modes & 1u) != 0, (p->modes & 2u) != 0, (p->modes & 12u) != 0};
        for (auto *f : e->files)
            for (int k = 0; k < 3; ++k)
                if (need[k]) PC_TRY(build_center_stream(e, f, k, e->param));
    }
    PC_TRY(refresh_file_views(e));
    if (!center && !dense && !p->d_hist.p) {
        const int rc = p->d_hist_own.reserve(std::max<size_t>((size_t)p->npos * p->rows * sizeof(uint32_t), 8));
        p->d_hist.p = p->d_hist_own.p;
        PC_TRY(rc);
    }
    return p->d_out.reserve(std::max<size_t>((size_t)p->out_elems * 8, 8));
}

int ensure_dense_tables(pc_engine *e, pc_plan *p, const StagedFile *sf);

int count_clear(pc_engine *e, pc_plan *p, const CountCall &c, const StagedFile *dense, int *path) {
    const bool center = e->kind == PC_MAP_CENTER;
    PC_TRY(mark(e, 0));
    int dense_path = PC_DENSE_PATH_NONE;
    if (dense) {
        PC_TRY(ensure_dense_tables(e, p, dense));
        const bool chunks = p->chunks_ok && p->dchunks_id == dense->did && !e->knobs.dense_items && ((uintptr_t)p->d_out.p & 127u) == 0;
        dense_path = chunks ? PC_DENSE_PATH_CHUNKS : PC_DENSE_PATH_ITEMS;
    }
    *path = dense_path;
    if (dense_path != PC_DENSE_PATH_NONE) {
        if (dense_path == PC_DENSE_PATH_ITEMS && p->covered != p->out_elems && p->out_elems)
            HIP_TRY(hipMemsetAsync(p->d_out.p, 0, (size_t)p->out_elems * 8, e->stream));
        return mark(e, 1);
    }
    if ((p->has_sums || p->out_needs_zero || p->covered != p->out_elems) && p->out_elems)
        HIP_TRY(hipMemsetAsync(p->d_out.p, 0, (size_t)p->out_elems * 8, e->stream));
    p->hist_lazy = !center && (int64_t)c.hist_bytes >= e->knobs.hist_lazy_bytes && !e->knobs.hist_memset;
    if (!center && c.hist_bytes && !p->hist_clean && !p->hist_lazy) {
        HIP_TRY(hipMemsetAsync(p->d_hist.p, 0, c.hist_bytes, e->stream));
        p->hist_clean = true;
    }
    return mark(e, 1);
}

int count_single(pc_engine *e, pc_plan *p, const CountCall &c) {
    const HistLds s = hist_lds_shape(e);
    const size_t lds = ((size_t)p->max_slots * p->rows * p->G + s.table_words) * sizeof(uint32_t);
    if (lds > e->max_lds)
        return fail(PC_ERR_ARG, "pc_count: the window needs %zu bytes of LDS, the device offers %zu per workgroup (too many rows)", lds, e->max_lds);
    const FileView fv0 = e->files[0]->view();
    PC_TRY(mark(e, 2));
    dispatch_hist<false>(e->kind, c.outmode, [&](auto K, auto O) {
        constexpr int k = decltype(K)::value, o = decltype(O)::value;
        hipLaunchKernelGGL((k_hist_point<k, o, kHistWG, false, false, true>), dim3(1), dim3(kHistWG), lds, e->stream, p->d_pieces.p, p->d_opieces.p,
                           fv0, fv0, e->d_files.p, (const WorkItem *)p->d_tiles.p, p->d_wcounters.p, p->d_tile_items.p, c.mp, p->G, p->max_slots,
                           s.tab_lo, s.tab_n, s.fast_lo, s.fast_hi, (uint32_t *)p->d_hist.p, (int64_t)e->Ws(), (typename OutT_<o>::type *)p->d_out.p,
                           e->norm_sum, (uint32_t)e->Wg(), (uint32_t)e->Wr(), (const FileRange *)nullptr, c.nfiles, Tile{}, OutPiece{}, (uint32_t *)nullptr, 0u);
    });
    PC_TRY(mark(e, 3));
    return mark(e, 4);
}

struct WorkLists {
    int64_t cap = 0, cap_small = 0;
    int small_g = 0;
    pc_plan::WorkKey key;
    HistLds shape;
    size_t lds = 0, lds_small = 0;
    unsigned grid = 0, grid_front = 0, grid_small = 0;
    uint32_t launched[3] = {0xffffffffu, 0xffffffffu, 0xffffffffu};
};

int size_work_lists(pc_engine *e, pc_plan *p, const CountCall &c, WorkLists &w) {
    const int nfiles = c.nfiles, G = p->G;
    const int64_t R = e->knobs.work_r;
    const int64_t pile = e->knobs.pile ? e->knobs.pile : 12 * R;
    const int halo = std::max(std::max(e->W(), e->Ws()), std::max(e->Wg(), e->Wr()));
    const int tiles_per_window = p->rows > 1 ? std::max(1, __builtin_popcount(p->modes)) : 1;
    const double windows_per_record = (1.0 + (double)(halo + 127) / (double)G) * (double)tiles_per_window;
    w.cap = (int64_t)c.ntiles * nfiles + (int64_t)(2.0 * windows_per_record * (double)c.nrec / (double)R) + nfiles + 64;
    const bool b16 = e->kind == PC_MAP_STRAT5;
    if (b16) {
        int64_t nxl = 0, ngp = 0;
        for (auto *f : e->files) { nxl += f->nxlong; ngp += f->ngap; }
        w.cap += (int64_t)(6.0 * windows_per_record * (double)(c.nrec + c.nextra + ngp) / (double)R) +
                 (int64_t)c.ntiles * nfiles * (4 + 2 * (nxl / R));
    }
    if (w.cap >= (int64_t)0xffffffffu) return fail(PC_ERR_ARG, "pc_count: work list too large");
    PC_TRY(p->d_work.reserve((size_t)w.cap));
    const bool sparse_plan = (double)p->npos < 0.25 * (double)c.ntiles * (double)G;
    w.small_g = ((p->rows == 1 || e->knobs.small_rows) && sparse_plan && !e->knobs.no_small) ? std::min(e->knobs.small_g, G) : 0;
    w.cap_small = w.small_g ? (int64_t)c.ntiles * nfiles : 0;
    PC_TRY(p->d_work_small.reserve((size_t)std::max<int64_t>(w.cap_small, 1)));
    if (nfiles > 1) {
        PC_TRY(p->d_chain.reserve((size_t)w.cap * (size_t)(nfiles - 1)));
        PC_TRY(p->d_chain_small.reserve((size_t)std::max<int64_t>(w.cap_small, 1) * (size_t)(nfiles - 1)));
    }
    pc_plan::WorkKey &key = w.key;
    key.generation = e->work_generation; key.nfiles = nfiles; key.G = G; key.Wg = e->Wg(); key.Ws = e->Ws(); key.Wr = e->Wr();
    key.small_g = w.small_g; key.R = R; key.pile = pile; key.small_n = e->knobs.small_n; key.cap = w.cap;
    w.shape = hist_lds_shape(e);
    const size_t slot_words = (size_t)p->max_slots * p->rows;
    w.lds = (((slot_words * G) >> (b16 ? 1 : 0)) + w.shape.table_words) * sizeof(uint32_t);
    w.lds_small = (((slot_words * w.small_g) >> (b16 ? 1 : 0)) + w.shape.table_words) * sizeof(uint32_t);
    return PC_OK;
}

int ensure_readback(uint32_t **host, hipEvent_t *ev, size_t words) {
    if (*host) return PC_OK;
    HIP_TRY(hipHostMalloc((void **)host, words * sizeof(uint32_t), hipHostMallocDefault));
    HIP_TRY(hipEventCreateWithFlags(ev, hipEventDisableTiming));
    return PC_OK;
}

int ensure_work_counts(pc_plan *p) { return ensure_readback(&p->h_work_counts, &p->ev_work_counts, 8); }

void take_work_counts(pc_plan *p) {
    for (int k = 0; k < 3; ++k) p->work_counts[k] = p->h_work_counts[k];
    p->work_merged = p->h_work_counts[4];
    p->work_counts_known = true;
}

int canonical_for_plan(pc_engine *e, pc_plan *p, const CountCall &c, const HistLds &shape, StagedFile **canon) {
    using namespace pcstage;
    *canon = nullptr;
    const bool point = e->kind == PC_MAP_FIVE || e->kind == PC_MAP_THREE || e->kind == PC_MAP_VAR5;
    if (e->knobs.no_canon || c.nfiles != 1 || !point || p->rows != 1 || (p->modes & ~3u) != 0u || p->modes == 0u) return PC_OK;
    StagedFile *sf = e->files[0];
    if (sf->n <= 0 || !sf->nlin) return PC_OK;
    CanonSig sig;
    sig.kind = e->kind; sig.param = e->kind == PC_MAP_VAR5 ? 0 : e->param;
    sig.filt_on = e->filt_on; sig.filt_min = e->filt_on ? e->filt_min : 0; sig.filt_max = e->filt_on ? e->filt_max : -1;
    sig.fast_lo = shape.fast_lo; sig.fast_hi = shape.fast_hi; sig.Ws = e->Ws(); sig.words_gen = sf->words_gen;
    if (e->kind == PC_MAP_VAR5) { sig.fw = e->h_fw; sig.rc = e->h_rc; }
    if (!(sf->ksig_valid && sf->ksig == sig)) {
        sf->ksig_valid = false;
        sf->kn = -1;
        pccanon::RuleIn r;
        r.kind = e->kind == PC_MAP_FIVE ? 0 : (e->kind == PC_MAP_THREE ? 1 : 3);
        r.param = e->param; r.table_len = (int)std::min<size_t>((size_t)e->table_len, std::min(e->h_fw.size(), e->h_rc.size()));
        r.fw = e->h_fw.data(); r.rc = e->h_rc.data();
        r.filt_on = e->filt_on; r.filt_min = e->filt_min; r.filt_max = e->filt_max;
        r.fast_lo = shape.fast_lo; r.fast_hi = shape.fast_hi;
        const pccanon::CanonRule cr = pccanon::canon_rule(r);
        if (cr.usable && pccanon::canon_fits_halo(cr, sig.Ws)) {
            PoolScope pool_scope(&e->pool);
            hipStream_t st = e->stream;
            const int64_t nlin = (int64_t)sf->nlin;
            PC_TRY(sf->klin_tab.reserve((size_t)nlin + 1));
            PC_TRY(sf->kshift.reserve(2 * pccanon::kLenSlots));
            DevBuf<uint8_t> d_scan;
            size_t tb = 0;
            HIP_TRY(hipcub::DeviceScan::ExclusiveSum(nullptr, tb, sf->klin_tab.p, sf->klin_tab.p, (int)nlin + 1, st));
            PC_TRY(d_scan.reserve(std::max<size_t>(tb, 16)));
            HIP_TRY(hipMemcpyAsync(sf->kshift.p, cr.shift, sizeof(cr.shift), hipMemcpyHostToDevice, st));
            HIP_TRY(hipMemsetAsync(sf->klin_tab.p + nlin, 0, 4, st));
            const int back = pccanon::canon_buckets_back(cr, kLinShift);
            const uint32_t lc0 = (uint32_t)cr.Lc[0] << 4, lc1 = ((uint32_t)cr.Lc[1] << 4) | 4u;
            hipLaunchKernelGGL((k_canon_buckets<false>), dim3((unsigned)std::min<int64_t>(nlin, kCanonMaxGrid)), dim3(256), 0, st, sf->stream.p, sf->lin_tab.p, sf->lin_off.p, e->ntid, nlin,
                               sf->kshift.p, back, lc0, lc1, sf->klin_tab.p, (uint32_t *)nullptr);
            hipError_t he = hipcub::DeviceScan::ExclusiveSum(d_scan.p, tb, sf->klin_tab.p, sf->klin_tab.p, (int)nlin + 1, st);
            uint32_t total = 0;
            if (he == hipSuccess) he = hipMemcpyAsync(&total, sf->klin_tab.p + nlin, 4, hipMemcpyDeviceToHost, st);
            if (he == hipSuccess) he = hipGetLastError();
            if (he == hipSuccess) he = hipStreamSynchronize(st);
            if (he != hipSuccess) return fail(PC_ERR_HIP, "building the canonical stream failed: %s", hipGetErrorString(he));
            const int64_t replaces = sf->cn >= 0 ? sf->cn : sf->n;
            if ((double)total <= e->knobs.compact_keep * (double)replaces) {
                PC_TRY(sf->kstream.reserve((size_t)total + 8));
                hipLaunchKernelGGL((k_canon_buckets<true>), dim3((unsigned)std::min<int64_t>(nlin, kCanonMaxGrid)), dim3(256), 0, st, sf->stream.p, sf->lin_tab.p, sf->lin_off.p, e->ntid, nlin,
                                   sf->kshift.p, back, lc0, lc1, sf->klin_tab.p, sf->kstream.p);
                hipLaunchKernelGGL(k_canon_pad, dim3(1), dim3(64), 0, st, sf->klin_tab.p, nlin, sf->kstream.p);
                HIP_TRY(hipGetLastError());
                sf->kn = (int64_t)total;
            }
        }
        if (sf->kn < 0) { sf->kstream.release(); sf->klin_tab.release(); }
        sf->ksig = sig;
        sf->ksig_valid = true;
        sf->kid += 1;
    }
    if (sf->kn >= 0) *canon = sf;
    return PC_OK;
}

FileView hist_view(pc_engine *e, const StagedFile *canon) {
    FileView v = e->files[0]->view();
    if (canon) { v.cstream = canon->kstream.p; v.clin_tab = canon->klin_tab.p; }
    return v;
}

int build_work_lists(pc_engine *e, pc_plan *p, const CountCall &c, const WorkLists &w, const StagedFile *canon) {
    hipStream_t st = e->stream;
    const int ntiles = c.ntiles;
    if (!p->wcounters_zero) HIP_TRY(hipMemsetAsync(p->d_wcounters.p, 0, 8 * sizeof(uint32_t), st));
    if (!p->tile_items_zero) HIP_TRY(hipMemsetAsync(p->d_tile_items.p, 0, ((size_t)ntiles + 1) * sizeof(uint32_t), st));
    p->wcounters_zero = false;
    p->tile_items_zero = false;
    const int64_t nwin = ntiles;
    const int lanes = (nwin * 16 <= e->knobs.ranges_cg16_max && !e->knobs.ranges_cg1) ? 16 : 1;
    dispatch_int<16, 1>(lanes, [&](auto CG) {
        hipLaunchKernelGGL((k_tile_ranges<decltype(CG)::value>), dim3((unsigned)((nwin * lanes + kRangesWG - 1) / kRangesWG)), dim3(kRangesWG), 0, st, p->d_tiles.p, ntiles,
                           hist_view(e, canon), e->d_files.p, c.nfiles, p->G, e->Wg(), e->Ws(), e->Wr(), w.key.R, w.key.pile, p->d_work.p, p->d_wcounters.p, p->d_tile_items.p, (uint32_t)w.cap,
                           p->d_work_small.p, w.small_g, w.key.small_n, e->knobs.debug_work, p->d_chain.p, p->d_chain_small.p, e->kind == PC_MAP_STRAT5 ? 1 : 0);
    });
    if (p->hist_lazy)
        hipLaunchKernelGGL(k_clear_split, dim3((unsigned)((ntiles + kClearPerWG - 1) / kClearPerWG)), dim3(kWG), 0, st, p->d_tiles.p, ntiles,
                           p->d_pieces.p, p->d_tile_items.p, p->d_wcounters.p, p->rows, (uint32_t *)p->d_hist.p, (int64_t)p->npos);
    p->work_key = w.key;
    p->work_valid = true;
    p->work_counts_known = false;
    p->guard_pending = true;
    p->work_counts_generation = 0;
    const int64_t spare = w.cap + w.cap_small - nwin;
    if (ntiles >= 4096 && spare >= e->knobs.first_sync_spare && !e->knobs.test_stale_counts && !e->knobs.debug_work) {
        PC_TRY(ensure_work_counts(p));
        HIP_TRY(hipMemcpyAsync(p->h_work_counts, p->d_wcounters.p, 8 * sizeof(uint32_t), hipMemcpyDeviceToHost, st));
        HIP_TRY(hipStreamSynchronize(st));
        take_work_counts(p);
        p->work_counts_generation = e->work_generation;
    }
    return PC_OK;
}

void choose_grids(pc_engine *e, pc_plan *p, const CountCall &c, WorkLists &w) {
    w.grid = w.grid_front = (unsigned)w.cap;
    w.grid_small = (unsigned)w.cap_small;
    if (c.ntiles < 4096 || p->work_counts_generation != e->work_generation) return;
    if (p->h_work_counts && !p->work_counts_known && hipEventQuery(p->ev_work_counts) == hipSuccess) take_work_counts(p);
    if (!p->work_counts_known) return;
    const uint32_t nh = p->work_counts[0], nl = p->work_counts[1] - ((e->knobs.test_stale_counts && p->work_counts[1]) ? 1u : 0u), ns = p->work_counts[2];
    if ((uint64_t)nh + nl <= (uint64_t)w.cap && (int64_t)ns <= w.cap_small) {
        w.grid_front = nh;
        w.grid = std::max(1u, nh + nl);
        w.grid_small = ns;
        w.launched[0] = nh; w.launched[1] = nl; w.launched[2] = ns;
        p->exact_grid_used = true;
    }
}

int launch_hist(pc_engine *e, pc_plan *p, const CountCall &c, const WorkLists &w, const StagedFile *canon) {
    const HistLds &s = w.shape;
    const int nfiles = c.nfiles;
    const FileView fv0 = hist_view(e, canon);
    const FileView fv1 = nfiles > 1 ? e->files[1]->view() : fv0;
    hipStream_t st = e->stream, st_small = e->side_stream;
    if (w.cap_small) {
        HIP_TRY(hipEventRecord(e->ev_fork, st));
        HIP_TRY(hipStreamWaitEvent(st_small, e->ev_fork, 0));
    }
    dispatch_hist<true>(e->kind, c.outmode, [&](auto K, auto O) {
        dispatch_int<0, 1>(nfiles > 1, [&](auto M) {
            constexpr int k = decltype(K)::value, o = decltype(O)::value;
            constexpr bool m = decltype(M)::value != 0;
            typename OutT_<o>::type *out = (typename OutT_<o>::type *)p->d_out.p;
            hipLaunchKernelGGL((k_hist_point<k, o, kHistWG, false, m>), dim3(w.grid), dim3(kHistWG), w.lds, st, p->d_pieces.p,
                               p->d_opieces.p, fv0, fv1, e->d_files.p, p->d_work.p, p->d_wcounters.p, p->d_tile_items.p, c.mp,
                               p->G, p->max_slots, s.tab_lo, s.tab_n, s.fast_lo, s.fast_hi, (uint32_t *)p->d_hist.p, p->npos, out,
                               e->norm_sum, (uint32_t)w.cap, w.grid_front, p->d_chain.p, nfiles, Tile{}, OutPiece{}, (uint32_t *)nullptr, 0u);
            if (w.cap_small && w.grid_small)
                hipLaunchKernelGGL((k_hist_point<k, o, 64, true, m>), dim3(w.grid_small), dim3(64), w.lds_small, st_small,
                                   p->d_pieces.p, p->d_opieces.p, fv0, fv1, e->d_files.p, p->d_work_small.p,
                                   p->d_wcounters.p, p->d_tile_items.p, c.mp, w.small_g, p->max_slots, s.tab_lo, s.tab_n, s.fast_lo, s.fast_hi,
                                   (uint32_t *)p->d_hist.p, p->npos, out, e->norm_sum, (uint32_t)w.cap_small, w.grid_small,
                                   p->d_chain_small.p, nfiles, Tile{}, OutPiece{}, (uint32_t *)nullptr, 0u);
        });
    });
    if (w.cap_small) {
        HIP_TRY(hipEventRecord(e->ev_join, st_small));
        HIP_TRY(hipStreamWaitEvent(st, e->ev_join, 0));
    }
    return PC_OK;
}

void merge_windows(pc_engine *e, pc_plan *p, const CountCall &c, const WorkLists &w) {
    if (w.launched[0] != 0xffffffffu && p->work_merged == 0 && !e->knobs.test_stale_counts) return;
    const int split_per_wg = kWG;
    dispatch_int<0, 1, 2>(c.outmode, [&](auto O) {
        constexpr int o = decltype(O)::value;
        hipLaunchKernelGGL((k_gather_split<o>), dim3((unsigned)((c.ntiles + split_per_wg - 1) / split_per_wg)), dim3(kWG), 0, e->stream,
                           p->d_tiles.p, c.ntiles, split_per_wg, p->d_pieces.p,
                           p->d_opieces.p, p->d_tile_items.p, p->d_wcounters.p, p->rows, (uint32_t *)p->d_hist.p, p->npos,
                           (typename OutT_<o>::type *)p->d_out.p, e->norm_sum, w.launched[0], w.launched[1], w.launched[2], (uint32_t)w.cap, e->d_counters.p + 12);
    });
}

int read_work_counts(pc_engine *e, pc_plan *p, const CountCall &c, const WorkLists &w) {
    hipStream_t st = e->stream;
    if (c.ntiles >= 4096) {
        PC_TRY(ensure_work_counts(p));
        if (p->work_counts_generation != e->work_generation) {
            p->work_counts_known = false;
            HIP_TRY(hipMemcpyAsync(p->h_work_counts, p->d_wcounters.p, 8 * sizeof(uint32_t), hipMemcpyDeviceToHost, st));
            HIP_TRY(hipEventRecord(p->ev_work_counts, st));
            p->work_counts_generation = e->work_generation;
        }
    }
    if (e->knobs.debug_work) {
        uint32_t c4[4] = {0, 0, 0, 0};
        HIP_TRY(hipMemcpyAsync(c4, p->d_wcounters.p, sizeof(c4), hipMemcpyDeviceToHost, st));
        HIP_TRY(hipStreamSynchronize(st));
        fprintf(stderr, "[work] tiles %d: heavy %u light %u small %u, long-span candidates %u (capacity %lld, G %d, R %lld)\n", c.ntiles,
                c4[0], c4[1], c4[2], c4[3], (long long)w.cap, p->G, (long long)w.key.R);
    }
    return PC_OK;
}

int count_lists(pc_engine *e, pc_plan *p, const CountCall &c) {
    WorkLists w;
    PC_TRY(size_work_lists(e, p, c, w));
    StagedFile *canon = nullptr;
    PC_TRY(canonical_for_plan(e, p, c, w.shape, &canon));
    w.key.canon = canon ? canon->kid : 0;
    if (!(p->work_valid && p->work_key == w.key) || e->knobs.debug_work) PC_TRY(build_work_lists(e, p, c, w, canon));
    PC_TRY(mark(e, 2));
    if (w.lds > e->max_lds)
        return fail(PC_ERR_ARG, "pc_count: the window needs %zu bytes of LDS, the device offers %zu per workgroup (too many rows)", w.lds, e->max_lds);
    choose_grids(e, p, c, w);
    PC_TRY(launch_hist(e, p, c, w, canon));
    PC_TRY(mark(e, 3));
    PC_TRY(mark(e, 4));
    merge_windows(e, p, c, w);
    return read_work_counts(e, p, c, w);
}

DenseSig dense_sig(const pc_engine *e, const StagedFile *sf) {
    DenseSig sig;
    sig.kind = e->kind; sig.param = e->kind == PC_MAP_VAR5 ? 0 : e->param;
    sig.filt_on = e->filt_on; sig.filt_min = e->filt_on ? e->filt_min : 0; sig.filt_max = e->filt_on ? e->filt_max : -1;
    sig.words_gen = sf->words_gen; sig.applied = sf->applied;
    if (e->kind == PC_MAP_VAR5) { sig.fw = e->h_fw; sig.rc = e->h_rc; }
    return sig;
}

std::atomic<uint64_t> g_dense_id{0};

int build_dense_vector(pc_engine *e, StagedFile *sf, const DenseSig &sig) {
    using namespace pcdense;
    sf->dsig_valid = false;
    const int ntid = e->ntid;
    const int64_t cells = sf->dcells;
    std::vector<int32_t> tid;
    std::vector<int64_t> start, end, off, stride;
    std::vector<uint8_t> strand;
    std::vector<int8_t> step;
    for (int t = 0; t < ntid; ++t)
        for (int s = 0; s < 2 && sf->dext[(size_t)t] > 0; ++s) {
            tid.push_back(t); start.push_back(0); end.push_back(sf->dext[(size_t)t]); strand.push_back(s ? PC_STRAND_REV : PC_STRAND_FWD);
            off.push_back(sf->dcell_off[(size_t)(2 * t + s)]); step.push_back(1); stride.push_back(0);
        }
    pc_plan *ip = nullptr;
    PC_TRY(pc_plan_create(e, (int64_t)tid.size(), tid.data(), start.data(), end.data(), strand.data(), off.data(), step.data(), stride.data(), cells, 1, &ip));
    ip->no_dense = true;
    const int norm_on = e->norm_on, prof_level = e->prof_level;
    e->norm_on = 0; e->prof_level = 0;
    int rc = pc_count(e, ip, PC_OUT_INT64);
    e->norm_on = norm_on; e->prof_level = prof_level;
    auto narrow = [&]() -> int {
        PoolScope pool_scope(&e->pool);
        hipStream_t st = e->stream;
        DevBuf<uint32_t> d_n, d_key, d_val;
        DevBuf<uint8_t> d_tmp;
        PC_TRY(sf->dense.reserve((size_t)cells + 8));
        PC_TRY(sf->d_dext.upload(sf->dext, st));
        PC_TRY(sf->d_dcell_off.upload(sf->dcell_off, st));
        PC_TRY(d_n.reserve(2));
        HIP_TRY(hipMemsetAsync(d_n.p, 0, 8, st));
        const unsigned grid = (unsigned)((cells + 255) / 256);
        const int64_t *src = (const int64_t *)ip->d_out.p;
        hipLaunchKernelGGL(k_dense_narrow, dim3(grid), dim3(256), 0, st, src, cells, sf->dense.p, d_n.p);
        uint32_t n_ovf = 0;
        HIP_TRY(hipGetLastError());
        HIP_TRY(hipMemcpyAsync(&n_ovf, d_n.p, 4, hipMemcpyDeviceToHost, st));
        HIP_TRY(hipStreamSynchronize(st));
        if (n_ovf) {
            size_t tb = 0;
            HIP_TRY(hipcub::DeviceRadixSort::SortPairs(nullptr, tb, (const uint32_t *)nullptr, (uint32_t *)nullptr, (const uint32_t *)nullptr, (uint32_t *)nullptr, (int)n_ovf, 0, 32, st));
            PC_TRY(d_key.reserve(n_ovf)); PC_TRY(d_val.reserve(n_ovf)); PC_TRY(d_tmp.reserve(std::max<size_t>(tb, 16)));
            PC_TRY(sf->dovf_key.reserve(n_ovf)); PC_TRY(sf->dovf_val.reserve(n_ovf));
            hipLaunchKernelGGL(k_dense_overflow, dim3(grid), dim3(256), 0, st, src, cells, d_n.p + 1, n_ovf, d_key.p, d_val.p);
            HIP_TRY(hipcub::DeviceRadixSort::SortPairs(d_tmp.p, tb, d_key.p, sf->dovf_key.p, d_val.p, sf->dovf_val.p, (int)n_ovf, 0, 32, st));
            HIP_TRY(hipGetLastError());
            HIP_TRY(hipStreamSynchronize(st));
        }
        sf->dn_ovf = n_ovf;
        return PC_OK;
    };
    if (rc == PC_OK) rc = narrow();
    (void)pc_plan_destroy(ip);
    PC_TRY(rc);
    sf->dsig = sig;
    sf->dsig_valid = true;
    sf->did = ++g_dense_id;
    return PC_OK;
}

int dense_for_plan(pc_engine *e, pc_plan *p, const CountCall &c, StagedFile **dense) {
    *dense = nullptr;
    pcdense::PlanIn in;
    in.nfiles = c.nfiles;
    in.point_rule = e->kind == PC_MAP_FIVE || e->kind == PC_MAP_THREE || e->kind == PC_MAP_VAR5;
    in.rows = p->rows; in.modes = p->modes; in.has_sums = p->has_sums;
    in.forbidden = e->knobs.no_dense || p->no_dense;
    if (!pcdense::plan_conditions(in)) return PC_OK;
    StagedFile *sf = e->files[0];
    if (sf->n <= 0 || !sf->nlin || sf->tid_end.size() != (size_t)e->ntid) return PC_OK;
    if (sf->dcells < 0) {
        sf->dext.resize((size_t)e->ntid);
        sf->dcell_off.resize(2 * (size_t)e->ntid + 1);
        for (int t = 0; t < e->ntid; ++t) sf->dext[(size_t)t] = pcdense::extent(0, sf->tid_end[(size_t)t]);
        sf->dcells = pcdense::layout(e->ntid, sf->dext.data(), sf->dcell_off.data());
    }
    in.cells = sf->dcells;
    if (!pcdense::build_fits(in.cells) || in.cells >= (int64_t)0xffffffffu) return PC_OK;
    StagedFile *canon = nullptr;
    PC_TRY(canonical_for_plan(e, p, c, hist_lds_shape(e), &canon));
    in.stream_entries = canon ? canon->kn : (sf->cn >= 0 ? sf->cn : sf->n);
    const bool ok = pcdense::eligible(in);
    if (e->knobs.dense_debug)
        fprintf(stderr, "[dense] cells %lld (%lld bytes) against %lld entries of the %s stream (%lld bytes): %s\n", (long long)in.cells,
                (long long)(in.cells * pcdense::kBytesPerCell), (long long)in.stream_entries, canon ? "canonical" : (sf->cn >= 0 ? "compact" : "record"),
                (long long)(in.stream_entries * 4), ok ? "vector" : "window kernels");
    if (!ok) return PC_OK;
    const DenseSig sig = dense_sig(e, sf);
    if (!(sf->dsig_valid && sf->dsig == sig)) PC_TRY(build_dense_vector(e, sf, sig));
    *dense = sf;
    return PC_OK;
}

int build_dense_chunks(pc_engine *e, pc_plan *p, const StagedFile *sf, const GatherSeg *gsegs, const int32_t *tid, const uint8_t *strand) {
    using namespace pcdense;
    p->chunks_ok = false;
    const size_t n = (size_t)p->nseg, nchunks = (size_t)chunks_of(p->out_elems);
    if (!n || !nchunks || !spans_fit((int64_t)n, p->covered) || nchunks >= (size_t)0x7fffffffu) return PC_OK;
    hipStream_t st = e->stream;
    DevBuf<uint64_t> d_key, d_key2;
    DevBuf<uint32_t> d_idx, d_idx2, d_cnt, d_at, d_first, d_nof, d_flag;
    DevBuf<uint8_t> d_tmp;
    d_key.pool = d_key2.pool = d_idx.pool = d_idx2.pool = d_cnt.pool = d_at.pool = d_first.pool = d_nof.pool = d_flag.pool = d_tmp.pool = &e->pool;
    size_t sort_b = 0, scan_b = 0;
    const uint64_t nokey = (uint64_t)p->out_elems;
    const int key_bits = bits_for(nokey);
    HIP_TRY(hipcub::DeviceRadixSort::SortPairs(nullptr, sort_b, (const uint64_t *)nullptr, (uint64_t *)nullptr, (const uint32_t *)nullptr, (uint32_t *)nullptr, (int)n, 0, key_bits, st));
    HIP_TRY(hipcub::DeviceScan::ExclusiveSum(nullptr, scan_b, (const uint32_t *)nullptr, (uint32_t *)nullptr, (int)n + 1, st));
    PC_TRY(d_key.reserve(n)); PC_TRY(d_key2.reserve(n)); PC_TRY(d_idx.reserve(n)); PC_TRY(d_idx2.reserve(n));
    PC_TRY(d_cnt.reserve(n + 1)); PC_TRY(d_at.reserve(n + 1)); PC_TRY(d_first.reserve(nchunks)); PC_TRY(d_nof.reserve(nchunks)); PC_TRY(d_flag.reserve(2));
    PC_TRY(d_tmp.reserve(std::max<size_t>(std::max(sort_b, scan_b), 16)));
    const unsigned g = (unsigned)((n + 255) / 256);
    hipLaunchKernelGGL(k_chunk_keys, dim3(g), dim3(256), 0, st, gsegs, (int64_t)n, nokey, d_key.p, d_idx.p);
    HIP_TRY(hipcub::DeviceRadixSort::SortPairs(d_tmp.p, sort_b, d_key.p, d_key2.p, d_idx.p, d_idx2.p, (int)n, 0, key_bits, st));
    HIP_TRY(hipMemsetAsync(d_cnt.p + n, 0, 4, st));
    HIP_TRY(hipMemsetAsync(d_flag.p, 0, 8, st));
    hipLaunchKernelGGL(k_chunk_count, dim3(g), dim3(256), 0, st, gsegs, d_key2.p, d_idx2.p, (int64_t)n, nokey, d_cnt.p, d_flag.p);
    HIP_TRY(hipcub::DeviceScan::ExclusiveSum(d_tmp.p, scan_b, d_cnt.p, d_at.p, (int)n + 1, st));
    PC_TRY(p->d_dspans.reserve(2 * n + (size_t)(p->covered / kChunk) + 1));
    PC_TRY(p->d_dchunks.reserve(nchunks));
    HIP_TRY(hipMemsetAsync(d_nof.p, 0, nchunks * 4, st));
    HIP_TRY(hipMemsetAsync(d_first.p, 0, nchunks * 4, st));
    hipLaunchKernelGGL(k_chunk_spans, dim3(g), dim3(256), 0, st, gsegs, tid, strand, d_key2.p, d_idx2.p, (int64_t)n, nokey, e->ntid, sf->d_dcell_off.p, sf->d_dext.p, d_at.p,
                       p->d_dspans.p, d_first.p, d_nof.p);
    hipLaunchKernelGGL(k_chunk_descs, dim3((unsigned)((nchunks + 255) / 256)), dim3(256), 0, st, p->d_dspans.p, d_first.p, d_nof.p, d_flag.p, (int64_t)nchunks, p->d_dchunks.p);
    HIP_TRY(hipGetLastError());
    uint32_t overlap = 0;
    HIP_TRY(hipMemcpyAsync(&overlap, d_flag.p, 4, hipMemcpyDeviceToHost, st));
    HIP_TRY(hipStreamSynchronize(st));
    if (overlap) return PC_OK;
    p->chunks_ok = true;
    return PC_OK;
}

int ensure_dense_tables(pc_engine *e, pc_plan *p, const StagedFile *sf) {
    using namespace pcdense;
    const bool need_items = p->ditems_id != sf->did, need_chunks = !e->knobs.dense_items && p->dchunks_id != sf->did;
    if (!need_items && !need_chunks) return PC_OK;
    hipStream_t st = e->stream;
    const size_t n = (size_t)p->nseg;
    if (need_items) { p->ditems_id = 0; p->n_ditems = 0; }
    if (need_chunks) { p->dchunks_id = 0; p->chunks_ok = false; }
    DevBuf<int32_t> d_tid;
    DevBuf<uint8_t> d_strand, d_tmp;
    DevBuf<uint32_t> d_cnt, d_at;
    d_tid.pool = d_strand.pool = d_tmp.pool = d_cnt.pool = d_at.pool = &e->pool;
    const GatherSeg *gsegs = p->gpu_built ? p->d_gsegs_own.p : p->d_gsegs.p;
    const int32_t *tid = nullptr;
    const uint8_t *strand = nullptr;
    if (p->gpu_built) {
        const PlanInputLayout L(n);
        tid = (const int32_t *)(p->d_inputs.p + L.at_tid); strand = p->d_inputs.p + L.at_strand;
    } else {
        PC_TRY(d_tid.upload(p->h_tid, st)); PC_TRY(d_strand.upload(p->h_strand, st));
        tid = d_tid.p; strand = d_strand.p;
    }
    if (need_items) {
        uint32_t total = 0;
        if (n) {
            size_t tb = 0;
            HIP_TRY(hipcub::DeviceScan::ExclusiveSum(nullptr, tb, (const uint32_t *)nullptr, (uint32_t *)nullptr, (int)n + 1, st));
            PC_TRY(d_cnt.reserve(n + 1)); PC_TRY(d_at.reserve(n + 1)); PC_TRY(d_tmp.reserve(std::max<size_t>(tb, 16)));
            const unsigned g = (unsigned)((n + 255) / 256);
            HIP_TRY(hipMemsetAsync(d_cnt.p + n, 0, 4, st));
            hipLaunchKernelGGL(k_dense_seg_items, dim3(g), dim3(256), 0, st, gsegs, (int64_t)n, d_cnt.p);
            HIP_TRY(hipcub::DeviceScan::ExclusiveSum(d_tmp.p, tb, d_cnt.p, d_at.p, (int)n + 1, st));
            HIP_TRY(hipMemcpyAsync(&total, d_at.p + n, 4, hipMemcpyDeviceToHost, st));
            HIP_TRY(hipStreamSynchronize(st));
            PC_TRY(p->d_ditems.reserve(std::max<size_t>(total, 1)));
            if (total) hipLaunchKernelGGL(k_dense_items, dim3(g), dim3(256), 0, st, gsegs, tid, strand, (int64_t)n, e->ntid, sf->d_dcell_off.p, sf->d_dext.p, d_at.p, p->d_ditems.p);
            HIP_TRY(hipGetLastError());
        }
        p->n_ditems = total;
    }
    if (need_chunks && n && build_dense_chunks(e, p, sf, gsegs, tid, strand) != PC_OK) { p->chunks_ok = false; (void)hipGetLastError(); }
    HIP_TRY(hipStreamSynchronize(st));
    if (need_items) p->ditems_id = sf->did;
    if (need_chunks) p->dchunks_id = sf->did;
    return PC_OK;
}

int count_dense(pc_engine *e, pc_plan *p, const CountCall &c, const StagedFile *sf, int path) {
    PC_TRY(mark(e, 2));
    if (path == PC_DENSE_PATH_CHUNKS)
        dispatch_int<0, 1, 2>(c.outmode, [&](auto O) {
            constexpr int o = decltype(O)::value;
            hipLaunchKernelGGL((pcdense::k_dense_gather_chunks<o>), dim3((unsigned)pcdense::chunks_of(p->out_elems)), dim3(pcdense::kGatherWG), 0, e->stream,
                               p->d_dchunks.p, p->d_dspans.p, sf->dense.p, sf->dovf_key.p, sf->dovf_val.p, sf->dn_ovf, (typename OutT_<o>::type *)p->d_out.p,
                               (int64_t)p->out_elems, e->norm_sum);
        });
    else if (p->n_ditems)
        dispatch_int<0, 1, 2>(c.outmode, [&](auto O) {
            constexpr int o = decltype(O)::value;
            hipLaunchKernelGGL((pcdense::k_dense_gather<o>), dim3((unsigned)pcdense::batches_of(p->n_ditems)), dim3(pcdense::kGatherWG), 0, e->stream, p->d_ditems.p,
                               (uint32_t)p->n_ditems, sf->dense.p, sf->dovf_key.p, sf->dovf_val.p, sf->dn_ovf, (typename OutT_<o>::type *)p->d_out.p, e->norm_sum);
        });
    PC_TRY(mark(e, 3));
    return mark(e, 4);
}

int reserve_center(pc_engine *e, pc_plan *p) {
    const size_t nchunks = p->n_cchunks, nfiles = e->files.size();
    if (kCenterCap * (int64_t)nchunks >= (int64_t)1 << kSubShift) return fail(PC_ERR_ARG, "pc_count: too many positions for the center rule");
    PC_TRY(p->d_corder.reserve((size_t)kCenterCap * nchunks));
    PC_TRY(p->d_ccand.reserve(nchunks));
    PC_TRY(p->d_cranges.reserve(nchunks * nfiles));
    PC_TRY(p->d_crec.reserve(nchunks * nfiles));
    PC_TRY(p->d_crows.reserve(nchunks * nfiles * (size_t)(2 * kCenterRows)));
    PC_TRY(p->d_ccounts.reserve(8));
    PC_TRY(e->d_cvalh.reserve(256));
    return p->d_cslots.reserve(2 * nchunks * nfiles);
}

int build_center_dispatch(pc_engine *e, pc_plan *p, int W) {
    hipStream_t st = e->stream;
    const int nfiles = (int)e->files.size();
    const int64_t nchunks = (int64_t)p->n_cchunks;
    p->center_nfiles = nfiles;
    HIP_TRY(hipMemsetAsync(p->d_ccounts.p, 0, 8 * sizeof(uint32_t), st));
    unsigned long long *total = (unsigned long long *)(p->d_ccounts.p + 2);
    const unsigned wgs = (unsigned)((nchunks + kRangesWG - 1) / kRangesWG);
    hipLaunchKernelGGL(k_center_weigh, dim3(wgs), dim3(kRangesWG), 0, st, p->d_cchunks.p, nchunks, e->d_files.p, nfiles, W,
                       p->d_ccand.p, p->d_cranges.p, p->d_crec.p, p->d_crows.p, total);
    const int ck1 = e->knobs.center_t1, ck2 = e->knobs.center_t2;
    hipLaunchKernelGGL(k_center_order, dim3(wgs), dim3(kRangesWG), 0, st, p->d_ccand.p, nchunks, total, e->knobs.center_floor,
                       (int64_t)2048, ck1, ck2, p->d_corder.p, p->d_ccounts.p);
    hipLaunchKernelGGL(k_center_slots, dim3((unsigned)((2 * nchunks + kRangesWG - 1) / kRangesWG)), dim3(kRangesWG), 0, st, p->d_cchunks.p, nchunks,
                       e->d_files.p, nfiles, W, p->d_corder.p, p->d_ccounts.p, p->d_cranges.p, p->d_crec.p, p->d_crows.p, p->d_opieces.p,
                       p->d_cslots.p, (unsigned long long *)(p->d_ccounts.p + 4));
    p->center_generation = e->work_generation;
    p->center_W = W;
    PC_TRY(ensure_readback(&p->h_center_counts, &p->ev_center_counts, 2));
    p->center_counts_known = false;
    HIP_TRY(hipMemcpyAsync(p->h_center_counts, p->d_ccounts.p, 2 * sizeof(uint32_t), hipMemcpyDeviceToHost, st));
    HIP_TRY(hipEventRecord(p->ev_center_counts, st));
    return PC_OK;
}

void launch_center2(pc_engine *e, pc_plan *p, const CountCall &c, int W, unsigned long long *dbg, size_t dbg_slots) {
    Center2Ctx c2;
    StagedFile *sf0 = e->files[0];
    c2.slots = p->d_cslots.p;
    c2.indirect = 0u;
    for (int k = 0; k < 3; ++k) {
        c2.ent[k] = sf0->cs_n[k] >= 0 ? sf0->cs_ent[k].p : nullptr;
        if (sf0->len_max > 255) c2.indirect |= 1u << k;
    }
    c2.files = e->d_files.p; c2.nfiles = c.nfiles; c2.file0 = sf0->view(); c2.mp = c.mp; c2.W = W; c2.inv = e->d_inv.p; c2.invh = e->d_invh.p; c2.cvalh = e->d_cvalh.p;
    c2.counters = p->d_ccounts.p;
    c2.known = p->center_counts_known ? 1u : 0u; c2.n_heavy = p->center_counts[0]; c2.n_light = p->center_counts[1];
    c2.opieces = p->d_opieces.p; c2.out = (double *)p->d_out.p; c2.norm_sum = e->norm_sum; c2.norm_on = e->norm_on ? 1 : 0;
    c2.dbg = dbg; c2.dbg_cap = (uint32_t)dbg_slots;
    uint64_t g2;
    if (p->center_counts_known) {
        const uint64_t n8 = ((uint64_t)p->center_counts[1] + 7) >> 3;
        g2 = (uint64_t)p->center_counts[0] + 8 * ((n8 + PC_CENTER_PER_WAVE - 1) / PC_CENTER_PER_WAVE);
    } else g2 = 2 * (uint64_t)p->n_cchunks + 8;
    const dim3 cg2((unsigned)std::max<uint64_t>(g2, 1));
    bool general = false;
    for (auto *f : e->files) general |= f->len_max > 255 || f->n + f->nrun >= ((int64_t)1 << 28);
    dispatch_int<0, 1>(dbg != nullptr, [&](auto D) {
        dispatch_int<0, 1>(general, [&](auto G) {
            dispatch_int<0, 1>(c.nfiles > 1, [&](auto M) {
                hipLaunchKernelGGL((k_center2<decltype(D)::value != 0, decltype(G)::value != 0, decltype(M)::value != 0>), cg2, dim3(64), (size_t)e->knobs.center_lds, e->stream, c2);
            });
        });
    });
}

int report_center_debug(pc_engine *e, pc_plan *p, int W, const unsigned long long *d_dbg, size_t dbg_slots) {
    std::vector<unsigned long long> h(2 * dbg_slots), h_slots(dbg_slots);
    HIP_TRY(hipStreamSynchronize(e->stream));
    HIP_TRY(hipMemcpy(h.data(), d_dbg, h.size() * 8, hipMemcpyDeviceToHost));
    HIP_TRY(hipMemcpy(h_slots.data(), d_dbg + h.size(), h_slots.size() * 8, hipMemcpyDeviceToHost));
    e->center_steps = 0; e->center_waves = 0;
    unsigned long long t0 = ~0ull, t1 = 0, sum = 0, steps_heavy = 0, steps_pers = 0, n_heavy_w = 0, n_pers_w = 0;
    const size_t n_front = p->n_cchunks;
    std::vector<std::pair<unsigned long long, size_t>> byd;
    for (size_t i = 0; i < dbg_slots; ++i)
        if (h[2 * i]) {
            e->center_steps += (int64_t)h_slots[i]; e->center_waves += 1;
            const bool pers = i >= n_front;
            (pers ? steps_pers : steps_heavy) += h_slots[i];
            (pers ? n_pers_w : n_heavy_w) += 1;
            t0 = std::min(t0, h[2 * i + 1]); t1 = std::max(t1, h[2 * i + 1] + h[2 * i]);
            sum += h[2 * i];
            byd.emplace_back(h[2 * i], i);
        }
    if (e->knobs.center_debug != 0) {
        fprintf(stderr, "[center] replay steps: %llu in %llu waves of the heavy entries, %llu in %llu waves of the light ones\n", steps_heavy, n_heavy_w,
                steps_pers, n_pers_w);
        fprintf(stderr, "[center] W %d: launch span %llu ticks (100 MHz: %.3f ms), summed wave time %llu ticks = %.1f x the span\n", W, t1 - t0,
                (t1 - t0) / 1e5, sum, (double)sum / (double)std::max<unsigned long long>(t1 - t0, 1));
        const int nb = 20;
        std::vector<double> occ(nb, 0.0);
        const double span = (double)std::max<unsigned long long>(t1 - t0, 1);
        for (size_t i = 0; i < dbg_slots; ++i)
            if (h[2 * i]) {
                const double a = (double)(h[2 * i + 1] - t0) / span * nb, b = (double)(h[2 * i + 1] + h[2 * i] - t0) / span * nb;
                for (int k = std::max(0, (int)a); k < nb && k < b; ++k) occ[(size_t)k] += std::min(b, k + 1.0) - std::max(a, (double)k);
            }
        fprintf(stderr, "[center] resident waves per twentieth of the launch:");
        for (int k = 0; k < nb; ++k) fprintf(stderr, " %.0f", occ[(size_t)k]);
        fprintf(stderr, "\n");
        std::sort(byd.rbegin(), byd.rend());
        for (size_t k = 0; k < std::min<size_t>(byd.size(), 8); ++k) {
            const size_t i = byd[k].second;
            fprintf(stderr, "[center]   slot %zu (%s): %.3f ms, started at %.3f ms, %llu steps\n", i,
                    i >= n_front ? "light" : "heavy", byd[k].first / 1e5, (h[2 * i + 1] - t0) / 1e5, h_slots[i]);
        }
        if (!byd.empty()) {
            const size_t i = byd.back().second;
            fprintf(stderr, "[center]   shortest: slot %zu: %.3f ms, %llu steps\n", i, byd.back().first / 1e5, h_slots[i]);
        }
    }
    return PC_OK;
}

int count_center(pc_engine *e, pc_plan *p, const CountCall &c) {
    PC_TRY(mark(e, 2));
    if (p->n_cchunks > 0) {
        const int W = e->W();
        PC_TRY(reserve_center(e, p));
        hipLaunchKernelGGL(k_center_vals, dim3(1), dim3(256), 0, e->stream, c.mp, e->d_invh.p, e->d_cvalh.p);
        if (p->center_generation != e->work_generation || p->center_W != W || p->center_nfiles != c.nfiles) {
            PC_TRY(build_center_dispatch(e, p, W));
        } else if (!p->center_counts_known && hipEventQuery(p->ev_center_counts) == hipSuccess) {
            p->center_counts[0] = p->h_center_counts[0];
            p->center_counts[1] = p->h_center_counts[1];
            p->center_counts_known = true;
        }
        DevBuf<unsigned long long> d_dbg;
        const bool dbg_on = e->knobs.center_debug != 0 || e->want_center_steps;
        const size_t dbg_slots = (size_t)kCenterCap * p->n_cchunks;
        if (dbg_on) {
            PC_TRY(d_dbg.reserve(3 * dbg_slots));
            HIP_TRY(hipMemsetAsync(d_dbg.p, 0, 3 * dbg_slots * 8, e->stream));
        }
        launch_center2(e, p, c, W, d_dbg.p, dbg_slots);
        if (dbg_on) PC_TRY(report_center_debug(e, p, W, d_dbg.p, dbg_slots));
    }
    PC_TRY(mark(e, 3));
    return mark(e, 4);
}

int count_finish(pc_engine *e, pc_plan *p, const CountCall &c) {
    PC_TRY(mark(e, 5));
    HIP_TRY(hipGetLastError());
    p->last_dtype = c.out_dtype;
    p->counted = true;
    p->rle_runs = -1;
    e->timing_valid = e->prof_level > 0;
    e->timed_level = e->prof_level;
    e->last_alg_bytes = c.nrec * 8 + (c.nextra > 0 ? c.nextra * 8 : 0) + p->nseg * 24 + p->covered * 8;
    return PC_OK;
}

}

extern "C" {

int pc_count(pc_engine *e, pc_plan *p, int out_dtype) {
    PC_TRY(count_validate(e, p, out_dtype));
    HIP_TRY(hipSetDevice(e->device));
    const bool center = e->kind == PC_MAP_CENTER;
    CountCall c;
    c.out_dtype = out_dtype;
    c.outmode = e->norm_on ? 2 : (out_dtype == PC_OUT_FLOAT64 ? 1 : 0);
    c.nfiles = (int)e->files.size(); c.ntiles = (int)p->n_tiles;
    c.nrec = c.nextra = 0;
    for (auto *f : e->files) { c.nrec += f->n; c.nextra += f->nrun; }
    c.hist_bytes = center ? 0 : (size_t)p->npos * p->rows * sizeof(uint32_t);
    c.mp = e->params();
    const bool single = c.ntiles == 1 && c.nfiles == 1 && !e->knobs.debug_work && !e->knobs.no_single && e->kind != PC_MAP_STRAT5;
    StagedFile *dense = nullptr;
    if (!center && !single && c.ntiles > 0) PC_TRY(dense_for_plan(e, p, c, &dense));
    e->last_count_dense = dense != nullptr;
    PC_TRY(count_prepare(e, p, dense != nullptr));
    int dense_path = PC_DENSE_PATH_NONE;
    PC_TRY(count_clear(e, p, c, dense, &dense_path));
    e->last_dense_path = dense_path;
    if (center) PC_TRY(count_center(e, p, c));
    else if (dense) PC_TRY(count_dense(e, p, c, dense, dense_path));
    else if (single) PC_TRY(count_single(e, p, c));
    else if (c.ntiles > 0) PC_TRY(count_lists(e, p, c));
    else for (int k = 2; k <= 4; ++k) PC_TRY(mark(e, k));
    return count_finish(e, p, c);
}

int64_t pc_dense_cells(pc_engine *e, int file) {
    if (!e || file < 0 || file >= (int)e->files.size()) return -1;
    const StagedFile *sf = e->files[file];
    if (e->files.size() != 1 || e->knobs.no_dense || !e->last_count_dense) return -1;
    return (sf->dsig_valid && sf->dsig == dense_sig(e, sf)) ? sf->dcells : -1;
}

int pc_dense_path(pc_engine *e) { return e && pc_dense_cells(e, 0) >= 0 ? e->last_dense_path : PC_DENSE_PATH_NONE; }

int pc_sync(pc_engine *e) {
    if (!e) return fail(PC_ERR_ARG, "engine is NULL");
    HIP_TRY(hipSetDevice(e->device));
    HIP_TRY(hipStreamSynchronize(e->stream));
    return PC_OK;
}


static int check_grid_guard(pc_engine *e, pc_plan *p) {
    if (!p->exact_grid_used && !p->guard_pending) return PC_OK;
    uint32_t err = 0;
    HIP_TRY(hipMemcpyAsync(&err, e->d_counters.p + 12, sizeof(err), hipMemcpyDeviceToHost, e->stream));
    HIP_TRY(hipStreamSynchronize(e->stream));
    p->guard_pending = false;
    if (!err) return PC_OK;
    HIP_TRY(hipMemsetAsync(e->d_counters.p + 12, 0, sizeof(uint32_t), e->stream));
    p->work_counts_known = false;
    p->work_counts_generation = 0;
    p->exact_grid_used = false;
    p->work_valid = false;
    if (err & 2u)
        return fail(PC_ERR_STATE, "the work lists of this plan overflowed their capacity (results incomplete): an engine defect -- please report "
                                  "the annotation / alignment shape; PC_WORK_R changes the item size");
    return fail(PC_ERR_STATE, "a count of this plan queued more work items than the cached work counts launched (results incomplete); "
                              "the cache has been dropped -- count again");
}

static constexpr size_t kSmallRead = 256 * 1024;

int pc_read_counts(pc_engine *e, pc_plan *p, void *host_out, int64_t out_elems) {
    if (!e || !p || p->e != e || !p->counted) return fail(PC_ERR_STATE, "pc_read_counts: nothing counted yet");
    if (out_elems != p->out_elems || (out_elems > 0 && !host_out)) return fail(PC_ERR_ARG, "pc_read_counts: buffer size mismatch");
    HIP_TRY(hipSetDevice(e->device));
    PC_TRY(check_grid_guard(e, p));
    const size_t bytes = (size_t)out_elems * 8;
    const char *knob = getenv("PC_STAGE_SLICE");
    if (bytes >= 4 * TransferRing::kPiece || (bytes > 0 && knob)) {
        HIP_TRY(hipStreamSynchronize(e->stream));
        const std::vector<TransferJob> job{{host_out, p->d_out.p, bytes}};
        const size_t piece = knob ? (size_t)std::max<int64_t>(1, std::min<int64_t>(atoll(knob), 4096)) * 4096 : TransferRing::kPiece;
        return TransferRing::of(e->device).run(e->device, job, piece, knob != nullptr, true);
    }
    if (bytes > e->pinned.cap && e->pinned_busy) { HIP_TRY(hipEventSynchronize(e->ev_pinned)); e->pinned_busy = false; }
    if (bytes > 0 && bytes <= kSmallRead && e->pinned.reserve(bytes) == PC_OK) {
        HIP_TRY(hipMemcpyAsync(e->pinned.p, p->d_out.p, bytes, hipMemcpyDeviceToHost, e->stream));
        HIP_TRY(hipStreamSynchronize(e->stream));
        e->pinned_busy = false;
        memcpy(host_out, e->pinned.p, bytes);
        return PC_OK;
    }
    if (bytes > 0) HIP_TRY(hipMemcpyAsync(host_out, p->d_out.p, bytes, hipMemcpyDeviceToHost, e->stream));
    HIP_TRY(hipStreamSynchronize(e->stream));
    return PC_OK;
}

int pc_plan_coordinates(pc_engine *e, pc_plan *p, int64_t *host_out, int64_t out_elems) {
    if (!e || !p || p->e != e) return fail(PC_ERR_ARG, "pc_plan_coordinates: bad engine/plan");
    if (out_elems != p->out_elems || (out_elems > 0 && !host_out)) return fail(PC_ERR_ARG, "pc_plan_coordinates: buffer size mismatch");
    HIP_TRY(hipSetDevice(e->device));
    if (out_elems == 0) return PC_OK;
    DevBuf<int64_t> d;
    d.pool = &e->pool;
    int rc = d.reserve((size_t)out_elems);
    if (rc == PC_OK) rc = ensure_gather_tables(e, p);
    if (rc != PC_OK) return rc;
    hipStream_t st = e->stream;
    HIP_TRY(hipMemsetAsync(d.p, 0xff, (size_t)out_elems * 8, st));
    const unsigned grid = (unsigned)p->n_gchunks;
    if (grid) hipLaunchKernelGGL(k_coordinates, dim3(grid), dim3(kWG), 0, st, p->d_gsegs.p, p->d_gchunks.p, p->rows, d.p);
    HIP_TRY(hipGetLastError());
    HIP_TRY(hipMemcpyAsync(host_out, d.p, (size_t)out_elems * 8, hipMemcpyDeviceToHost, st));
    HIP_TRY(hipStreamSynchronize(st));
    return PC_OK;
}

void *pc_counts_device_ptr(pc_plan *p) { return p ? (void *)p->d_out.p : nullptr; }
void *pc_stream(pc_engine *e) { return e ? (void *)e->stream : nullptr; }
void *pc_total_device_ptr(pc_plan *p) { return p ? (void *)p->d_total.p : nullptr; }

int pc_total(pc_engine *e, pc_plan *p, void *host_out8) {
    if (!e || !p || p->e != e || !p->counted) return fail(PC_ERR_STATE, "pc_total: nothing counted yet");
    HIP_TRY(hipSetDevice(e->device));
    PC_TRY(check_grid_guard(e, p));
    hipStream_t st = e->stream;
    HIP_TRY(hipMemsetAsync(p->d_total.p, 0, 8, st));
    if (p->out_elems > 0) {
        if (p->last_dtype == PC_OUT_INT64) {
            hipLaunchKernelGGL(k_total_i64, dim3(1024), dim3(kWG), 0, st, (const int64_t *)p->d_out.p, p->out_elems, (int64_t *)p->d_total.p);
        } else {
            const int nb = 1024;
            PC_TRY(e->d_partial.reserve(nb));
            hipLaunchKernelGGL(k_total_f64_partial, dim3(nb), dim3(kWG), 0, st, (const double *)p->d_out.p, p->out_elems, e->d_partial.p);
            hipLaunchKernelGGL(k_total_f64_final, dim3(1), dim3(64), 0, st, e->d_partial.p, nb, (double *)p->d_total.p);
        }
    }
    if (host_out8) HIP_TRY(hipMemcpyAsync(host_out8, p->d_total.p, 8, hipMemcpyDeviceToHost, st));
    HIP_TRY(hipStreamSynchronize(st));
    return PC_OK;
}

int pc_rle(pc_engine *e, pc_plan *p, int64_t period, int64_t *n_runs) {
    if (!e || !p || p->e != e || !n_runs) return fail(PC_ERR_ARG, "pc_rle: bad arguments");
    if (!p->counted) return fail(PC_ERR_STATE, "pc_rle: nothing counted yet");
    if (period < 0) return fail(PC_ERR_ARG, "pc_rle: period must be >= 0");
    HIP_TRY(hipSetDevice(e->device));
    hipStream_t st = e->stream;
    const int64_t n = p->out_elems;
    p->rle_runs = 0;
    *n_runs = 0;
    if (n == 0) return PC_OK;
    const int64_t nwg = (n + kRleChunk - 1) / kRleChunk;
    int rc = p->d_rle_cnt.reserve((size_t)nwg);
    if (rc == PC_OK) rc = p->d_rle_base.reserve((size_t)nwg + 1);
    if (rc != PC_OK) return rc;
    const unsigned long long *v = (const unsigned long long *)p->d_out.p;
    hipLaunchKernelGGL(k_rle_count, dim3((unsigned)nwg), dim3(kWG), 0, st, v, n, period, p->d_rle_cnt.p);
    hipLaunchKernelGGL(k_rle_scan, dim3(1), dim3(kWG), 0, st, p->d_rle_cnt.p, nwg, p->d_rle_base.p, p->d_rle_base.p + nwg);
    int64_t total = 0;
    HIP_TRY(hipMemcpyAsync(&total, p->d_rle_base.p + nwg, sizeof(total), hipMemcpyDeviceToHost, st));
    HIP_TRY(hipStreamSynchronize(st));
    rc = p->d_rle_starts.reserve((size_t)std::max<int64_t>(total, 1));
    if (rc == PC_OK) rc = p->d_rle_values.reserve((size_t)std::max<int64_t>(total, 1));
    if (rc != PC_OK) return rc;
    hipLaunchKernelGGL(k_rle_write, dim3((unsigned)nwg), dim3(kWG), 0, st, v, n, period, p->d_rle_base.p, p->d_rle_starts.p,
                       p->d_rle_values.p);
    HIP_TRY(hipGetLastError());
    p->rle_runs = total;
    *n_runs = total;
    return PC_OK;
}

int pc_read_rle(pc_engine *e, pc_plan *p, int64_t *starts, void *values, int64_t n_runs) {
    if (!e || !p || p->e != e) return fail(PC_ERR_ARG, "pc_read_rle: bad arguments");
    if (p->rle_runs < 0) return fail(PC_ERR_STATE, "pc_read_rle: pc_rle has not run");
    if (n_runs != p->rle_runs || (n_runs > 0 && (!starts || !values))) return fail(PC_ERR_ARG, "pc_read_rle: expected %lld runs", (long long)p->rle_runs);
    HIP_TRY(hipSetDevice(e->device));
    if (n_runs > 0) {
        HIP_TRY(hipMemcpyAsync(starts, p->d_rle_starts.p, (size_t)n_runs * 8, hipMemcpyDeviceToHost, e->stream));
        HIP_TRY(hipMemcpyAsync(values, p->d_rle_values.p, (size_t)n_runs * 8, hipMemcpyDeviceToHost, e->stream));
    }
    HIP_TRY(hipStreamSynchronize(e->stream));
    return PC_OK;
}

int pc_set_profiling(pc_engine *e, int level) {
    if (!e) return fail(PC_ERR_ARG, "engine is NULL");
    if (level < 0 || level > 2) return fail(PC_ERR_ARG, "pc_set_profiling: level must be 0, 1 or 2");
    e->prof_level = level;
    e->timing_valid = false;
    return PC_OK;
}

// ... 342 lines not shown
```

### plastid_amd/engine.py

```python
import ctypes
import os
import weakref

import numpy as np

from . import _lib
from ._lib import (MAP_CENTER, MAP_FIVE, MAP_STRAT5, MAP_THREE, MAP_VAR5, OUT_FLOAT64, OUT_INT64,
                   check)

STRAND_CODE = {"\x00": 0, "+": 1, "-": 2, ".": 3}


def _ptr(a):
    return None if a is None else a.ctypes.data


def _c(a, dtype):
    return np.ascontiguousarray(a, dtype=dtype)


def release_cached_memory(device=0):
    check(_lib.load().pc_release_cached_memory(int(device)), "pc_release_cached_memory")


class Engine(object):

    def __init__(self, device=0):
        self._lib = _lib.load()
        h = ctypes.c_void_p()
        check(self._lib.pc_create(int(device), ctypes.byref(h)), "pc_create")
        self._h = h
        self.device = int(device)
        self._finalizer = weakref.finalize(self, self._lib.pc_destroy, h)
        self.rows = 1
        self.kind = None
        self.nfiles = 0
        self.ntid = 0
        self._state = {}

    def close(self):
        self._finalizer()

    def host_buffer(self, n, dtype=np.int64):
        dtype = np.dtype(dtype)
        nbytes = max(int(n), 0) * dtype.itemsize
        p = ctypes.c_void_p()
        check(self._lib.pc_host_alloc(self._h, nbytes, ctypes.byref(p)), "pc_host_alloc")
        raw = (ctypes.c_uint8 * max(nbytes, 1)).from_address(p.value)
        arr = np.frombuffer(raw, dtype=np.uint8, count=nbytes).view(dtype)
        lib, h, addr = self._lib, self._h, p.value
        fin = self._finalizer

        def release():
            if fin.alive:
                lib.pc_host_free(h, ctypes.c_void_p(addr))
        weakref.finalize(raw, release)
        return arr

    def clear_alignments(self):
        check(self._lib.pc_clear_alignments(self._h))
        self.nfiles = 0

    def add_alignment_file(self, packed, ntid=None):
        ntid = len(packed.references) if ntid is None else int(ntid)
        for name in ("pos", "alen", "flags", "nblk"):
            if len(getattr(packed, name)) != packed.n:
                raise ValueError("alignment array '%s' has %d entries, expected %d" % (name, len(getattr(packed, name)), packed.n))
        if len(packed.blk_start) != len(packed.blk_len):
            raise ValueError("run arrays blk_start / blk_len differ in length")
        if getattr(packed, "n_wide", 0):
            if len(packed.wide_alen) != packed.n_wide or len(packed.wide_nblk) != packed.n_wide:
                raise ValueError("wide_idx / wide_alen / wide_nblk differ in length")
            check(self._lib.pc_add_alignment_file_wide(
                self._h, packed.n, ntid, _ptr(packed.tid), _ptr(packed.pos), _ptr(packed.alen),
                _ptr(packed.flags), _ptr(packed.nblk), len(packed.blk_start), _ptr(packed.blk_start),
                _ptr(packed.blk_len), packed.n_wide, _ptr(packed.wide_idx), _ptr(packed.wide_alen), _ptr(packed.wide_nblk)))
        else:
            check(self._lib.pc_add_alignment_file(
                self._h, packed.n, ntid, _ptr(packed.tid), _ptr(packed.pos), _ptr(packed.alen),
                _ptr(packed.flags), _ptr(packed.nblk), len(packed.blk_start), _ptr(packed.blk_start),
                _ptr(packed.blk_len)))
        self.nfiles += 1
        self.ntid = ntid
        if getattr(packed, "flag16", None) is not None and getattr(packed, "mapq", None) is not None:
            self.set_alignment_sam(self.nfiles - 1, packed.flag16, packed.mapq)
        if getattr(packed, "nh", None) is not None:
            self.set_alignment_nh(self.nfiles - 1, packed.nh)

    def set_alignment_sam(self, file_index, flag16, mapq):
        flag16, mapq = _c(flag16, np.uint16), _c(mapq, np.uint8)
        if len(flag16) != len(mapq):
            raise ValueError("flag16 / mapq differ in length")
        check(self._lib.pc_set_alignment_sam(self._h, int(file_index), len(flag16), _ptr(flag16), _ptr(mapq)))

    def set_alignment_nh(self, file_index, nh):
        nh = _c(nh, np.uint16)
        check(self._lib.pc_set_alignment_nh(self._h, int(file_index), len(nh), _ptr(nh)))

    def set_nh_filter(self, max_nh=0):
        if self._state.get("nhfilter", 0) == int(max_nh):
            return
        check(self._lib.pc_set_nh_filter(self._h, int(max_nh)))
        self._state["nhfilter"] = int(max_nh)

    def set_flag_filter(self, require=0, exclude=0, min_mapq=0, enabled=True):
        key = (bool(enabled), int(require), int(exclude), int(min_mapq)) if enabled else (False, 0, 0, 0)
        if self._state.get("flagfilter", (False, 0, 0, 0)) == key:
            return
        check(self._lib.pc_set_flag_filter(self._h, 1 if enabled else 0, int(require), int(exclude), int(min_mapq)))
        self._state["flagfilter"] = key

    def set_alignments(self, files, ntid=None):
        self.clear_alignments()
        for f in files:
            self.add_alignment_file(f, ntid)

    def add_bam(self, path, regions=None, index=None, sort=False):
        import os
        from .bam import _no_sort_with_regions
        _no_sort_with_regions(sort, regions)
        if not os.path.isfile(path):
            raise IOError("No such file: %r" % (path,))
        mapped = ctypes.c_int64(0)
        if regions is not None:
            from .bam import resolve_regions, _index_path
            sp = resolve_regions(path, regions, index=_index_path(path, index, self))
            cb, ce = np.ascontiguousarray(sp["chunks"][:, 0]), np.ascontiguousarray(sp["chunks"][:, 1])
            rc = self._lib.pc_add_alignment_bam_chunks(self._h, os.fsencode(path), len(cb), _ptr(cb), _ptr(ce), len(sp["tid"]),
                                                       _ptr(sp["tid"]), _ptr(sp["beg"]), _ptr(sp["end"]), ctypes.byref(mapped))
        elif sort:
            from ._lib import PC_BAM_SORT
            rc = self._lib.pc_add_alignment_bam_path_flags(self._h, os.fsencode(path), PC_BAM_SORT, ctypes.byref(mapped))
        else:
            rc = self._lib.pc_add_alignment_bam_path(self._h, os.fsencode(path), ctypes.byref(mapped))
        check(rc)
        self.nfiles += 1
        return int(mapped.value)

    def add_sam(self, path, sort=False):
        import os
        from ._lib import PC_BAM_SORT
        path = os.fspath(path)
        if not os.path.isfile(path):
            raise IOError("No such file: %r" % (path,))
        mapped = ctypes.c_int64(0)
        check(self._lib.pc_add_alignment_sam_path_flags(self._h, os.fsencode(path), PC_BAM_SORT if sort else 0, ctypes.byref(mapped)))
        self.nfiles += 1
        return int(mapped.value)

    def num_records(self, file_index):
        return int(self._lib.pc_num_records(self._h, int(file_index)))

    def stream_entries(self, file_index):
        return int(self._lib.pc_stream_entries(self._h, int(file_index)))

    def canonical_entries(self, file_index):
        return int(self._lib.pc_canonical_entries(self._h, int(file_index)))

    def dense_cells(self, file_index):
        return int(self._lib.pc_dense_cells(self._h, int(file_index)))

    def dense_path(self):
        return {1: "items", 2: "chunks"}.get(int(self._lib.pc_dense_path(self._h)))

    def read_records(self, file_index, indices):
        idx = _c(indices, np.int64)
        n = len(idx)
        out = dict(tid=np.zeros(n, np.int32), pos=np.zeros(n, np.int32), alen=np.zeros(n, np.int32), reverse=np.zeros(n, np.uint8),
                   nblk=np.zeros(n, np.int32), flag16=np.zeros(n, np.uint16), mapq=np.zeros(n, np.uint8))
        check(self._lib.pc_read_records(self._h, int(file_index), n, _ptr(idx), _ptr(out["tid"]), _ptr(out["pos"]), _ptr(out["alen"]),
                                        _ptr(out["reverse"]), _ptr(out["nblk"]), _ptr(out["flag16"]), _ptr(out["mapq"])))
        cnt = np.where(out["alen"] > 0, np.maximum(out["nblk"], 1), 0).astype(np.int64)
        off = np.zeros(n + 1, np.int64)
        np.cumsum(cnt, out=off[1:])
        nr = int(off[-1])
        out["run_off"], out["run_start"], out["run_len"] = off, np.zeros(nr, np.int32), np.zeros(nr, np.int32)
        at = np.ascontiguousarray(off[:-1])
        check(self._lib.pc_read_record_runs(self._h, int(file_index), n, _ptr(idx), _ptr(at), nr, _ptr(out["run_start"]), _ptr(out["run_len"])))
        return out

    def update_flags(self, file_index, flags):
        flags = _c(flags, np.uint8)
        check(self._lib.pc_update_flags(self._h, int(file_index), len(flags), _ptr(flags)))

    def set_mapping(self, kind, param=0, fw=None, rc=None, min_len=25, max_len=35):
        if kind in (MAP_VAR5, MAP_STRAT5):
            fw = _c(fw, np.int32)
            rc = _c(rc, np.int32)
            n = len(fw)
            self._state.pop("map", None)
        else:
            fw = rc = None
            n = 0
            key = (int(kind), int(param))
            if self._state.get("map") == key:
                return
        check(self._lib.pc_set_mapping(self._h, int(kind), int(param), _ptr(fw), _ptr(rc), n,
                                       int(min_len), int(max_len)))
        self.kind = int(kind)
        self.rows = self._lib.pc_mapping_rows(self._h)
        if n == 0:
            self._state["map"] = key

    def set_size_filter(self, min_len=None, max_len=-1):
        if self._state.get("size") == (min_len, max_len):
            return
        if min_len is None:
            check(self._lib.pc_set_size_filter(self._h, 0, 0, -1))
        else:
            check(self._lib.pc_set_size_filter(self._h, 1, int(min_len), int(max_len)))
        self._state["size"] = (min_len, max_len)

    def set_normalize(self, enabled, total=1.0):
        if self._state.get("norm") == (bool(enabled), float(total)):
            return
        check(self._lib.pc_set_normalize(self._h, 1 if enabled else 0, float(total)))
        self._state["norm"] = (bool(enabled), float(total))

    def plan(self, tid, start, end, strand, out_off, out_step, row_stride, out_elems, rows=None):
        return Plan(self, tid, start, end, strand, out_off, out_step, row_stride, out_elems,
                    self.rows if rows is None else rows)

    def mapped_reads(self, file_index, rec_lo, rec_hi, tid, start, end, strand_code):
        n = int(rec_hi) - int(rec_lo)
        mask = np.zeros(max(n, 0), np.uint8)
        if n > 0:
            check(self._lib.pc_mapped_reads(self._h, int(file_index), int(rec_lo), int(rec_hi), int(tid),
                                            int(start), int(end), int(strand_code), _ptr(mask)))
        return mask

    def query_segment(self, tid, start, end, strand_code, reverse, dtype):
        out = np.empty(int(end) - int(start), dtype)
        check(self._lib.pc_query_segment(self._h, int(tid), int(start), int(end), int(strand_code), 1 if reverse else 0,
                                         OUT_FLOAT64 if dtype == np.float64 else OUT_INT64, out.ctypes.data))
        return out

    def export_batches(self, lengths, budget=None):
        lens = _c(lengths, np.int64)
        batch_of = np.zeros(max(len(lens), 1), np.int32)
        nb = ctypes.c_int(0)
        check(self._lib.pc_counts_export_batches(len(lens), _ptr(lens), int(budget or 0), _ptr(batch_of), ctypes.byref(nb)), "pc_counts_export_batches")
        return [[int(k) for k in np.nonzero(batch_of[:len(lens)] == b)[0]] for b in range(nb.value)]

    def counts_export_stats(self):
        stats, ms = np.zeros(4, np.int64), np.zeros(6, np.float64)
        check(self._lib.pc_counts_export_stats(self._h, _ptr(stats)))
        check(self._lib.pc_counts_export_timing(self._h, _ptr(ms)))
        return stats, ms

    def sync(self):
        check(self._lib.pc_sync(self._h))

    def set_profiling(self, level):
        check(self._lib.pc_set_profiling(self._h, int(level)))

    def last_timing(self):
        ms = np.zeros(6, np.float64)
        k = self._lib.pc_last_timing(self._h, _ptr(ms), 6)
        if k < 0:
            check(k)
        names = ("total", "worklist", "hist", "long", "gather", "zero")
        return dict(zip(names, ms.tolist()))

    def stream_probe(self, nbytes=1 << 30, iters=5):
        r = np.zeros(2, np.float64)
        check(self._lib.pc_stream_probe(self._h, int(nbytes), int(iters), r.ctypes.data, r.ctypes.data + 8))
        return float(r[0]), float(r[1])

    def reload_knobs(self):
        check(self._lib.pc_reload_knobs(self._h))

    def last_algorithmic_bytes(self):
        return int(self._lib.pc_last_algorithmic_bytes(self._h))

    def center_replay_steps(self, plan):
        steps, waves = ctypes.c_int64(0), ctypes.c_int64(0)
        check(self._lib.pc_center_replay_steps(self._h, plan._h, ctypes.byref(steps), ctypes.byref(waves)))
        return steps.value, waves.value

    def center_row_fill(self, plan):
        a, b = ctypes.c_int64(0), ctypes.c_int64(0)
        check(self._lib.pc_center_row_fill(self._h, plan._h, ctypes.byref(a), ctypes.byref(b)))
        return a.value, b.value

    @property
    def stream(self):
        return self._lib.pc_stream(self._h)


class Plan(object):

    def __init__(self, engine, tid, start, end, strand, out_off, out_step, row_stride, out_elems, rows):
        self.engine = engine
        self._lib = engine._lib
        self.tid = _c(tid, np.int32)
        self.start = _c(start, np.int64)
        self.end = _c(end, np.int64)
        self.strand = _c(strand, np.uint8)
        self.out_off = _c(out_off, np.int64)
        self.out_step = _c(out_step, np.int8)
        self.row_stride = _c(row_stride, np.int64)
        self.nseg = len(self.tid)
        for name in ("start", "end", "strand", "out_off", "out_step", "row_stride"):
            if len(getattr(self, name)) != self.nseg:
                raise ValueError("plan array '%s' has %d entries, expected %d" % (name, len(getattr(self, name)), self.nseg))
        self.out_elems = int(out_elems)
        self.rows = int(rows)
        h = ctypes.c_void_p()
        check(self._lib.pc_plan_create(
            engine._h, self.nseg, _ptr(self.tid), _ptr(self.start), _ptr(self.end), _ptr(self.strand),
            _ptr(self.out_off), _ptr(self.out_step), _ptr(self.row_stride), self.out_elems, self.rows,
            ctypes.byref(h)))
        self._h = h
        self._finalizer = weakref.finalize(self, Plan._destroy, self._lib, h, engine)
# ... 140 lines not shown
```

Baseline: 2103 billion reads/s.

## Share one dense count vector across all staged files and build chunk tables lazily

Moves the dense per-position count vector from each staged file to a single engine-level vector whose layout covers the joint extent of every file, so the dense gather path can also serve multi-file counts. The vector's signature now tracks each file's staging id and filter state. ensure_dense_tables now builds the chunk descriptors first and builds the item list only when the chunk path cannot be used, and it synchronises the stream only when device work was actually queued. The benchmark uses a single file, so the main effect there is skipping the redundant item-table build and one sync, at the cost of more complex cache invalidation logic.

```diff
diff --git a/include/plastid_counts.h b/include/plastid_counts.h
--- a/include/plastid_counts.h
+++ b/include/plastid_counts.h
@@ -7,7 +7,7 @@
 extern "C" {
 #endif
 
-#define PC_ABI_VERSION 23
+#define PC_ABI_VERSION 24
 
 typedef struct pc_engine pc_engine;
 typedef struct pc_plan pc_plan;
@@ -66,6 +66,7 @@
 int64_t pc_num_records(pc_engine *e, int file);
 int64_t pc_stream_entries(pc_engine *e, int file);
 int64_t pc_canonical_entries(pc_engine *e, int file);
+int64_t pc_dense_set_cells(pc_engine *e);
 int64_t pc_dense_cells(pc_engine *e, int file);
 #define PC_DENSE_PATH_NONE 0
 #define PC_DENSE_PATH_ITEMS 1
diff --git a/plastid_amd/_lib.py b/plastid_amd/_lib.py
--- a/plastid_amd/_lib.py
+++ b/plastid_amd/_lib.py
@@ -41,6 +41,7 @@
     "pc_stream_entries": (_i64, [_vp, _int]),
     "pc_canonical_entries": (_i64, [_vp, _int]),
     "pc_dense_cells": (_i64, [_vp, _int]),
+    "pc_dense_set_cells": (_i64, [_vp]),
     "pc_dense_path": (_int, [_vp]),
     "pc_read_records": (_int, [_vp, _int, _i64] + [_vp] * 8),
     "pc_read_record_runs": (_int, [_vp, _int, _i64, _vp, _vp, _i64, _vp, _vp]),
@@ -176,7 +177,7 @@
 
 PC_BAM_SORT = 1
 
-ABI_VERSION = 23
+ABI_VERSION = 24
 
 
 def load():
diff --git a/plastid_amd/csrc/dense_host.h b/plastid_amd/csrc/dense_host.h
--- a/plastid_amd/csrc/dense_host.h
+++ b/plastid_amd/csrc/dense_host.h
@@ -27,8 +27,25 @@
     return at;
 }
 
+inline int64_t joint_extent(int nfiles, const int64_t *const *tid_end, int t) {
+    int64_t far = 0;
+    for (int f = 0; f < nfiles; ++f)
+        if (tid_end[f] && tid_end[f][t] > far) far = tid_end[f][t];
+    return extent(0, far);
+}
+inline int64_t joint_layout(int ntid, int nfiles, const int64_t *const *tid_end, int64_t *ext, int64_t *cell_off) {
+    for (int t = 0; t < ntid; ++t) ext[t] = joint_extent(nfiles, tid_end, t);
+    return layout(ntid, ext, cell_off);
+}
+inline int64_t summed_entries(int nfiles, const int64_t *cn, const int64_t *n) {
+    int64_t sum = 0;
+    for (int f = 0; f < nfiles; ++f) sum += cn[f] >= 0 ? cn[f] : n[f];
+    return sum;
+}
+
 struct PlanIn {
     int nfiles = 0;
+    bool file_set = false;
     bool point_rule = false;
     int rows = 1;
     uint32_t modes = 0;
@@ -39,7 +56,7 @@
 };
 
 inline bool plan_conditions(const PlanIn &p) {
-    return !p.forbidden && p.nfiles == 1 && p.point_rule && p.rows == 1 && (p.modes & ~3u) == 0u && p.modes != 0u && !p.has_sums;
+    return !p.forbidden && (p.nfiles == 1 || (p.file_set && p.nfiles > 1)) && p.point_rule && p.rows == 1 && (p.modes & ~3u) == 0u && p.modes != 0u && !p.has_sums;
 }
 inline bool size_rule(int64_t cells, int64_t stream_entries) { return cells > 0 && cells * kBytesPerCell <= stream_entries * 4; }
 inline bool build_fits(int64_t cells) { return cells * 8 <= kBuildBlockCap; }
diff --git a/plastid_amd/csrc/plastid_counts.hip b/plastid_amd/csrc/plastid_counts.hip
--- a/plastid_amd/csrc/plastid_counts.hip
+++ b/plastid_amd/csrc/plastid_counts.hip
@@ -404,16 +404,22 @@
     }
 };
 
+struct DenseFileSig {
+    uint64_t sid = 0, words_gen = 0;
+    FilterState applied;
+    bool operator==(const DenseFileSig &o) const { return sid == o.sid && words_gen == o.words_gen && applied == o.applied; }
+};
 struct DenseSig {
     int kind = -1, param = 0, filt_on = 0, filt_min = 0, filt_max = -1;
-    uint64_t words_gen = 0;
-    FilterState applied;
+    std::vector<DenseFileSig> files;
     std::vector<int32_t> fw, rc;
     bool operator==(const DenseSig &o) const {
         return kind == o.kind && param == o.param && filt_on == o.filt_on && filt_min == o.filt_min && filt_max == o.filt_max &&
-               words_gen == o.words_gen && applied == o.applied && fw == o.fw && rc == o.rc;
+               files == o.files && fw == o.fw && rc == o.rc;
     }
 };
+
+std::atomic<uint64_t> g_staging_id{0};
 
 struct StagedFile {
     int64_t n = 0, nrun = 0, nlong = 0;
@@ -449,15 +455,7 @@
     CanonSig ksig;
     uint64_t kid = 0;
     std::vector<int64_t> tid_end;
-    std::vector<int64_t> dext, dcell_off;
-    int64_t dcells = -1;
-    DevBuf<int64_t> d_dext, d_dcell_off;
-    DevBuf<uint16_t> dense;
-    DevBuf<uint32_t> dovf_key, dovf_val;
-    uint32_t dn_ovf = 0;
-    bool dsig_valid = false;
-    DenseSig dsig;
-    uint64_t did = 0;
+    uint64_t sid = ++g_staging_id;
     size_t nlin = 0;
     int64_t nrunrec = 0;
     int Wr = 1;
@@ -503,6 +501,24 @@
         v.long_wide = nwide ? long_wide.p : nullptr; v.xlong_wide = nwide ? xlong_wide.p : nullptr;
         v.wide_rec = wide_rec.p; v.wide_val = wide_val.p; v.nwide = nwide;
         return v;
+    }
+};
+
+struct DenseVector {
+    std::vector<uint64_t> laid_for;
+    std::vector<int64_t> dext, dcell_off;
+    int64_t dcells = -1;
+    DevBuf<int64_t> d_dext, d_dcell_off;
+    DevBuf<uint16_t> dense;
+    DevBuf<uint32_t> dovf_key, dovf_val;
+    uint32_t dn_ovf = 0;
+    bool dsig_valid = false;
+    DenseSig dsig;
+    uint64_t did = 0;
+    void clear() {
+        laid_for.clear(); dext.clear(); dcell_off.clear();
+        dcells = -1; dn_ovf = 0; dsig_valid = false; dsig = DenseSig(); did = 0;
+        d_dext.release(); d_dcell_off.release(); dense.release(); dovf_key.release(); dovf_val.release();
     }
 };
 
@@ -588,6 +604,7 @@
     hipEvent_t ev_pinned = nullptr;
     hipEvent_t ev[8] = {};
     std::vector<StagedFile *> files;
+    DenseVector dvec;
     std::vector<pc_track *> tracks;
     std::vector<pc_bigwig_summary *> summaries;
     DevBuf<uint8_t> cx_text;
@@ -1278,6 +1295,7 @@
     destroy_summaries_of(e);
     for (auto *f : e->files) delete f;
     e->files.clear();
+    e->dvec.clear();
     for (auto &ev : e->ev)
         if (ev) (void)hipEventDestroy(ev);
     if (e->side_stream) { (void)hipStreamSynchronize(e->side_stream); (void)hipStreamDestroy(e->side_stream); }
@@ -1335,6 +1353,8 @@
     HIP_TRY(hipStreamSynchronize(e->stream));
     for (auto *f : e->files) delete f;
     e->files.clear();
+    e->dvec.clear();
+    e->last_count_dense = false;
     e->ntid = 0;
     e->files_dirty = true;
     e->work_generation += 1;
@@ -2337,16 +2357,16 @@
     return p->d_out.reserve(std::max<size_t>((size_t)p->out_elems * 8, 8));
 }
 
-int ensure_dense_tables(pc_engine *e, pc_plan *p, const StagedFile *sf);
-
-int count_clear(pc_engine *e, pc_plan *p, const CountCall &c, const StagedFile *dense, int *path) {
+int ensure_dense_tables(pc_engine *e, pc_plan *p, const DenseVector *dv);
+bool dense_by_chunks(const pc_engine *e, const pc_plan *p, const DenseVector *dv);
+
+int count_clear(pc_engine *e, pc_plan *p, const CountCall &c, const DenseVector *dense, int *path) {
     const bool center = e->kind == PC_MAP_CENTER;
     PC_TRY(mark(e, 0));
     int dense_path = PC_DENSE_PATH_NONE;
     if (dense) {
         PC_TRY(ensure_dense_tables(e, p, dense));
-        const bool chunks = p->chunks_ok && p->dchunks_id == dense->did && !e->knobs.dense_items && ((uintptr_t)p->d_out.p & 127u) == 0;
-        dense_path = chunks ? PC_DENSE_PATH_CHUNKS : PC_DENSE_PATH_ITEMS;
+        dense_path = dense_by_chunks(e, p, dense) ? PC_DENSE_PATH_CHUNKS : PC_DENSE_PATH_ITEMS;
     }
     *path = dense_path;
     if (dense_path != PC_DENSE_PATH_NONE) {
@@ -2645,30 +2665,33 @@
     return read_work_counts(e, p, c, w);
 }
 
-DenseSig dense_sig(const pc_engine *e, const StagedFile *sf) {
+DenseSig dense_sig(const pc_engine *e) {
     DenseSig sig;
     sig.kind = e->kind; sig.param = e->kind == PC_MAP_VAR5 ? 0 : e->param;
     sig.filt_on = e->filt_on; sig.filt_min = e->filt_on ? e->filt_min : 0; sig.filt_max = e->filt_on ? e->filt_max : -1;
-    sig.words_gen = sf->words_gen; sig.applied = sf->applied;
+    sig.files.resize(e->files.size());
+    for (size_t f = 0; f < e->files.size(); ++f) {
+        sig.files[f].sid = e->files[f]->sid; sig.files[f].words_gen = e->files[f]->words_gen; sig.files[f].applied = e->files[f]->applied;
+    }
     if (e->kind == PC_MAP_VAR5) { sig.fw = e->h_fw; sig.rc = e->h_rc; }
     return sig;
 }
 
 std::atomic<uint64_t> g_dense_id{0};
 
-int build_dense_vector(pc_engine *e, StagedFile *sf, const DenseSig &sig) {
+int build_dense_vector(pc_engine *e, DenseVector *dv, const DenseSig &sig) {
     using namespace pcdense;
-    sf->dsig_valid = false;
+    dv->dsig_valid = false;
     const int ntid = e->ntid;
-    const int64_t cells = sf->dcells;
+    const int64_t cells = dv->dcells;
     std::vector<int32_t> tid;
     std::vector<int64_t> start, end, off, stride;
     std::vector<uint8_t> strand;
     std::vector<int8_t> step;
     for (int t = 0; t < ntid; ++t)
-        for (int s = 0; s < 2 && sf->dext[(size_t)t] > 0; ++s) {
-            tid.push_back(t); start.push_back(0); end.push_back(sf->dext[(size_t)t]); strand.push_back(s ? PC_STRAND_REV : PC_STRAND_FWD);
-            off.push_back(sf->dcell_off[(size_t)(2 * t + s)]); step.push_back(1); stride.push_back(0);
+        for (int s = 0; s < 2 && dv->dext[(size_t)t] > 0; ++s) {
+            tid.push_back(t); start.push_back(0); end.push_back(dv->dext[(size_t)t]); strand.push_back(s ? PC_STRAND_REV : PC_STRAND_FWD);
+            off.push_back(dv->dcell_off[(size_t)(2 * t + s)]); step.push_back(1); stride.push_back(0);
         }
     pc_plan *ip = nullptr;
     PC_TRY(pc_plan_create(e, (int64_t)tid.size(), tid.data(), start.data(), end.data(), strand.data(), off.data(), step.data(), stride.data(), cells, 1, &ip));
@@ -2682,14 +2705,14 @@
         hipStream_t st = e->stream;
         DevBuf<uint32_t> d_n, d_key, d_val;
         DevBuf<uint8_t> d_tmp;
-        PC_TRY(sf->dense.reserve((size_t)cells + 8));
-        PC_TRY(sf->d_dext.upload(sf->dext, st));
-        PC_TRY(sf->d_dcell_off.upload(sf->dcell_off, st));
+        PC_TRY(dv->dense.reserve((size_t)cells + 8));
+        PC_TRY(dv->d_dext.upload(dv->dext, st));
+        PC_TRY(dv->d_dcell_off.upload(dv->dcell_off, st));
         PC_TRY(d_n.reserve(2));
         HIP_TRY(hipMemsetAsync(d_n.p, 0, 8, st));
         const unsigned grid = (unsigned)((cells + 255) / 256);
         const int64_t *src = (const int64_t *)ip->d_out.p;
-        hipLaunchKernelGGL(k_dense_narrow, dim3(grid), dim3(256), 0, st, src, cells, sf->dense.p, d_n.p);
+        hipLaunchKernelGGL(k_dense_narrow, dim3(grid), dim3(256), 0, st, src, cells, dv->dense.p, d_n.p);
         uint32_t n_ovf = 0;
         HIP_TRY(hipGetLastError());
         HIP_TRY(hipMemcpyAsync(&n_ovf, d_n.p, 4, hipMemcpyDeviceToHost, st));
@@ -2698,58 +2721,78 @@
             size_t tb = 0;
             HIP_TRY(hipcub::DeviceRadixSort::SortPairs(nullptr, tb, (const uint32_t *)nullptr, (uint32_t *)nullptr, (const uint32_t *)nullptr, (uint32_t *)nullptr, (int)n_ovf, 0, 32, st));
             PC_TRY(d_key.reserve(n_ovf)); PC_TRY(d_val.reserve(n_ovf)); PC_TRY(d_tmp.reserve(std::max<size_t>(tb, 16)));
-            PC_TRY(sf->dovf_key.reserve(n_ovf)); PC_TRY(sf->dovf_val.reserve(n_ovf));
+            PC_TRY(dv->dovf_key.reserve(n_ovf)); PC_TRY(dv->dovf_val.reserve(n_ovf));
             hipLaunchKernelGGL(k_dense_overflow, dim3(grid), dim3(256), 0, st, src, cells, d_n.p + 1, n_ovf, d_key.p, d_val.p);
-            HIP_TRY(hipcub::DeviceRadixSort::SortPairs(d_tmp.p, tb, d_key.p, sf->dovf_key.p, d_val.p, sf->dovf_val.p, (int)n_ovf, 0, 32, st));
+            HIP_TRY(hipcub::DeviceRadixSort::SortPairs(d_tmp.p, tb, d_key.p, dv->dovf_key.p, d_val.p, dv->dovf_val.p, (int)n_ovf, 0, 32, st));
             HIP_TRY(hipGetLastError());
             HIP_TRY(hipStreamSynchronize(st));
         }
-        sf->dn_ovf = n_ovf;
+        dv->dn_ovf = n_ovf;
         return PC_OK;
     };
     if (rc == PC_OK) rc = narrow();
     (void)pc_plan_destroy(ip);
     PC_TRY(rc);
-    sf->dsig = sig;
-    sf->dsig_valid = true;
-    sf->did = ++g_dense_id;
-    return PC_OK;
-}
-
-int dense_for_plan(pc_engine *e, pc_plan *p, const CountCall &c, StagedFile **dense) {
+    dv->dsig = sig;
+    dv->dsig_valid = true;
+    dv->did = ++g_dense_id;
+    return PC_OK;
+}
+
+int dense_for_plan(pc_engine *e, pc_plan *p, const CountCall &c, DenseVector **dense) {
     *dense = nullptr;
     pcdense::PlanIn in;
     in.nfiles = c.nfiles;
+    in.file_set = true;
     in.point_rule = e->kind == PC_MAP_FIVE || e->kind == PC_MAP_THREE || e->kind == PC_MAP_VAR5;
     in.rows = p->rows; in.modes = p->modes; in.has_sums = p->has_sums;
     in.forbidden = e->knobs.no_dense || p->no_dense;
     if (!pcdense::plan_conditions(in)) return PC_OK;
-    StagedFile *sf = e->files[0];
-    if (sf->n <= 0 || !sf->nlin || sf->tid_end.size() != (size_t)e->ntid) return PC_OK;
-    if (sf->dcells < 0) {
-        sf->dext.resize((size_t)e->ntid);
-        sf->dcell_off.resize(2 * (size_t)e->ntid + 1);
-        for (int t = 0; t < e->ntid; ++t) sf->dext[(size_t)t] = pcdense::extent(0, sf->tid_end[(size_t)t]);
-        sf->dcells = pcdense::layout(e->ntid, sf->dext.data(), sf->dcell_off.data());
-    }
-    in.cells = sf->dcells;
+    DenseVector *dv = &e->dvec;
+    const size_t nf = e->files.size();
+    bool any = false, same = dv->dcells >= 0 && dv->laid_for.size() == nf;
+    for (size_t f = 0; f < nf; ++f) {
+        const StagedFile *sf = e->files[f];
+        if (sf->n < 0 || (sf->n > 0 && (!sf->nlin || sf->tid_end.size() != (size_t)e->ntid))) return PC_OK;
+        any = any || sf->n > 0;
+        same = same && dv->laid_for[f] == sf->sid;
+    }
+    if (!any) return PC_OK;
+    if (!same) {
+        std::vector<const int64_t *> ends(nf);
+        dv->laid_for.resize(nf);
+        for (size_t f = 0; f < nf; ++f) {
+            ends[f] = e->files[f]->n > 0 ? e->files[f]->tid_end.data() : nullptr;
+            dv->laid_for[f] = e->files[f]->sid;
+        }
+        dv->dsig_valid = false;
+        dv->dext.resize((size_t)e->ntid);
+        dv->dcell_off.resize(2 * (size_t)e->ntid + 1);
+        dv->dcells = pcdense::joint_layout(e->ntid, (int)nf, ends.data(), dv->dext.data(), dv->dcell_off.data());
+    }
+    in.cells = dv->dcells;
     if (!pcdense::build_fits(in.cells) || in.cells >= (int64_t)0xffffffffu) return PC_OK;
     StagedFile *canon = nullptr;
     PC_TRY(canonical_for_plan(e, p, c, hist_lds_shape(e), &canon));
-    in.stream_entries = canon ? canon->kn : (sf->cn >= 0 ? sf->cn : sf->n);
+    if (canon) in.stream_entries = canon->kn;
+    else {
+        in.stream_entries = 0;
+        for (const StagedFile *sf : e->files) in.stream_entries += pcdense::summed_entries(1, &sf->cn, &sf->n);
+    }
     const bool ok = pcdense::eligible(in);
     if (e->knobs.dense_debug)
-        fprintf(stderr, "[dense] cells %lld (%lld bytes) against %lld entries of the %s stream (%lld bytes): %s\n", (long long)in.cells,
-                (long long)(in.cells * pcdense::kBytesPerCell), (long long)in.stream_entries, canon ? "canonical" : (sf->cn >= 0 ? "compact" : "record"),
+        fprintf(stderr, "[dense] %d file%s: cells %lld (%lld bytes) against %lld entries of the %s (%lld bytes): %s\n", c.nfiles, c.nfiles == 1 ? "" : "s",
+                (long long)in.cells, (long long)(in.cells * pcdense::kBytesPerCell), (long long)in.stream_entries,
+                canon ? "canonical stream" : (nf > 1 ? "files' streams" : (e->files[0]->cn >= 0 ? "compact stream" : "record stream")),
                 (long long)(in.stream_entries * 4), ok ? "vector" : "window kernels");
     if (!ok) return PC_OK;
-    const DenseSig sig = dense_sig(e, sf);
-    if (!(sf->dsig_valid && sf->dsig == sig)) PC_TRY(build_dense_vector(e, sf, sig));
-    *dense = sf;
-    return PC_OK;
-}
-
-int build_dense_chunks(pc_engine *e, pc_plan *p, const StagedFile *sf, const GatherSeg *gsegs, const int32_t *tid, const uint8_t *strand) {
+    const DenseSig sig = dense_sig(e);
+    if (!(dv->dsig_valid && dv->dsig == sig)) PC_TRY(build_dense_vector(e, dv, sig));
+    *dense = dv;
+    return PC_OK;
+}
+
+int build_dense_chunks(pc_engine *e, pc_plan *p, const DenseVector *dv, const GatherSeg *gsegs, const int32_t *tid, const uint8_t *strand) {
     using namespace pcdense;
     p->chunks_ok = false;
     const size_t n = (size_t)p->nseg, nchunks = (size_t)chunks_of(p->out_elems);
@@ -2778,7 +2821,7 @@
     PC_TRY(p->d_dchunks.reserve(nchunks));
     HIP_TRY(hipMemsetAsync(d_nof.p, 0, nchunks * 4, st));
     HIP_TRY(hipMemsetAsync(d_first.p, 0, nchunks * 4, st));
-    hipLaunchKernelGGL(k_chunk_spans, dim3(g), dim3(256), 0, st, gsegs, tid, strand, d_key2.p, d_idx2.p, (int64_t)n, nokey, e->ntid, sf->d_dcell_off.p, sf->d_dext.p, d_at.p,
+    hipLaunchKernelGGL(k_chunk_spans, dim3(g), dim3(256), 0, st, gsegs, tid, strand, d_key2.p, d_idx2.p, (int64_t)n, nokey, e->ntid, dv->d_dcell_off.p, dv->d_dext.p, d_at.p,
                        p->d_dspans.p, d_first.p, d_nof.p);
     hipLaunchKernelGGL(k_chunk_descs, dim3((unsigned)((nchunks + 255) / 256)), dim3(256), 0, st, p->d_dspans.p, d_first.p, d_nof.p, d_flag.p, (int64_t)nchunks, p->d_dchunks.p);
     HIP_TRY(hipGetLastError());
@@ -2790,14 +2833,16 @@
     return PC_OK;
 }
 
-int ensure_dense_tables(pc_engine *e, pc_plan *p, const StagedFile *sf) {
+bool dense_by_chunks(const pc_engine *e, const pc_plan *p, const DenseVector *dv) {
+    return p->chunks_ok && p->dchunks_id == dv->did && !e->knobs.dense_items && ((uintptr_t)p->d_out.p & 127u) == 0;
+}
+
+int ensure_dense_tables(pc_engine *e, pc_plan *p, const DenseVector *dv) {
     using namespace pcdense;
-    const bool need_items = p->ditems_id != sf->did, need_chunks = !e->knobs.dense_items && p->dchunks_id != sf->did;
-    if (!need_items && !need_chunks) return PC_OK;
+    const bool need_chunks = !e->knobs.dense_items && p->dchunks_id != dv->did;
+    if (!need_chunks && (dense_by_chunks(e, p, dv) || p->ditems_id == dv->did)) return PC_OK;
     hipStream_t st = e->stream;
     const size_t n = (size_t)p->nseg;
-    if (need_items) { p->ditems_id = 0; p->n_ditems = 0; }
-    if (need_chunks) { p->dchunks_id = 0; p->chunks_ok = false; }
     DevBuf<int32_t> d_tid;
     DevBuf<uint8_t> d_strand, d_tmp;
     DevBuf<uint32_t> d_cnt, d_at;
@@ -2805,52 +2850,71 @@
     const GatherSeg *gsegs = p->gpu_built ? p->d_gsegs_own.p : p->d_gsegs.p;
     const int32_t *tid = nullptr;
     const uint8_t *strand = nullptr;
+    bool busy = false;
     if (p->gpu_built) {
         const PlanInputLayout L(n);
         tid = (const int32_t *)(p->d_inputs.p + L.at_tid); strand = p->d_inputs.p + L.at_strand;
     } else {
+        busy = true;
         PC_TRY(d_tid.upload(p->h_tid, st)); PC_TRY(d_strand.upload(p->h_strand, st));
         tid = d_tid.p; strand = d_strand.p;
     }
-    if (need_items) {
+    auto body = [&]() -> int {
+        if (need_chunks) {
+            p->dchunks_id = 0; p->chunks_ok = false;
+            busy = true;
+            if (n && build_dense_chunks(e, p, dv, gsegs, tid, strand) != PC_OK) { p->chunks_ok = false; (void)hipGetLastError(); }
+            if (p->chunks_ok) busy = false;
+            p->dchunks_id = dv->did;
+        }
+        if (dense_by_chunks(e, p, dv) || p->ditems_id == dv->did) return PC_OK;
+        p->ditems_id = 0; p->n_ditems = 0;
         uint32_t total = 0;
         if (n) {
             size_t tb = 0;
             HIP_TRY(hipcub::DeviceScan::ExclusiveSum(nullptr, tb, (const uint32_t *)nullptr, (uint32_t *)nullptr, (int)n + 1, st));
             PC_TRY(d_cnt.reserve(n + 1)); PC_TRY(d_at.reserve(n + 1)); PC_TRY(d_tmp.reserve(std::max<size_t>(tb, 16)));
             const unsigned g = (unsigned)((n + 255) / 256);
+            busy = true;
             HIP_TRY(hipMemsetAsync(d_cnt.p + n, 0, 4, st));
             hipLaunchKernelGGL(k_dense_seg_items, dim3(g), dim3(256), 0, st, gsegs, (int64_t)n, d_cnt.p);
             HIP_TRY(hipcub::DeviceScan::ExclusiveSum(d_tmp.p, tb, d_cnt.p, d_at.p, (int)n + 1, st));
             HIP_TRY(hipMemcpyAsync(&total, d_at.p + n, 4, hipMemcpyDeviceToHost, st));
             HIP_TRY(hipStreamSynchronize(st));
+            busy = false;
             PC_TRY(p->d_ditems.reserve(std::max<size_t>(total, 1)));
-            if (total) hipLaunchKernelGGL(k_dense_items, dim3(g), dim3(256), 0, st, gsegs, tid, strand, (int64_t)n, e->ntid, sf->d_dcell_off.p, sf->d_dext.p, d_at.p, p->d_ditems.p);
+            if (total) {
+                busy = true;
+                hipLaunchKernelGGL(k_dense_items, dim3(g), dim3(256), 0, st, gsegs, tid, strand, (int64_t)n, e->ntid, dv->d_dcell_off.p, dv->d_dext.p, d_at.p, p->d_ditems.p);
+            }
             HIP_TRY(hipGetLastError());
         }
         p->n_ditems = total;
-    }
-    if (need_chunks && n && build_dense_chunks(e, p, sf, gsegs, tid, strand) != PC_OK) { p->chunks_ok = false; (void)hipGetLastError(); }
-    HIP_TRY(hipStreamSynchronize(st));
-    if (need_items) p->ditems_id = sf->did;
-    if (need_chunks) p->dchunks_id = sf->did;
-    return PC_OK;
-}
-
-int count_dense(pc_engine *e, pc_plan *p, const CountCall &c, const StagedFile *sf, int path) {
+        p->ditems_id = dv->did;
+        return PC_OK;
+    };
+    const int rc = body();
+    if (busy) {
+        const hipError_t he = hipStreamSynchronize(st);
+        if (rc == PC_OK) HIP_TRY(he);
+    }
+    return rc;
+}
+
+int count_dense(pc_engine *e, pc_plan *p, const CountCall &c, const DenseVector *dv, int path) {
     PC_TRY(mark(e, 2));
     if (path == PC_DENSE_PATH_CHUNKS)
         dispatch_int<0, 1, 2>(c.outmode, [&](auto O) {
             constexpr int o = decltype(O)::value;
             hipLaunchKernelGGL((pcdense::k_dense_gather_chunks<o>), dim3((unsigned)pcdense::chunks_of(p->out_elems)), dim3(pcdense::kGatherWG), 0, e->stream,
-                               p->d_dchunks.p, p->d_dspans.p, sf->dense.p, sf->dovf_key.p, sf->dovf_val.p, sf->dn_ovf, (typename OutT_<o>::type *)p->d_out.p,
+                               p->d_dchunks.p, p->d_dspans.p, dv->dense.p, dv->dovf_key.p, dv->dovf_val.p, dv->dn_ovf, (typename OutT_<o>::type *)p->d_out.p,
                                (int64_t)p->out_elems, e->norm_sum);
         });
     else if (p->n_ditems)
         dispatch_int<0, 1, 2>(c.outmode, [&](auto O) {
             constexpr int o = decltype(O)::value;
             hipLaunchKernelGGL((pcdense::k_dense_gather<o>), dim3((unsigned)pcdense::batches_of(p->n_ditems)), dim3(pcdense::kGatherWG), 0, e->stream, p->d_ditems.p,
-                               (uint32_t)p->n_ditems, sf->dense.p, sf->dovf_key.p, sf->dovf_val.p, sf->dn_ovf, (typename OutT_<o>::type *)p->d_out.p, e->norm_sum);
+                               (uint32_t)p->n_ditems, dv->dense.p, dv->dovf_key.p, dv->dovf_val.p, dv->dn_ovf, (typename OutT_<o>::type *)p->d_out.p, e->norm_sum);
         });
     PC_TRY(mark(e, 3));
     return mark(e, 4);
@@ -3030,7 +3094,7 @@
     c.hist_bytes = center ? 0 : (size_t)p->npos * p->rows * sizeof(uint32_t);
     c.mp = e->params();
     const bool single = c.ntiles == 1 && c.nfiles == 1 && !e->knobs.debug_work && !e->knobs.no_single && e->kind != PC_MAP_STRAT5;
-    StagedFile *dense = nullptr;
+    DenseVector *dense = nullptr;
     if (!center && !single && c.ntiles > 0) PC_TRY(dense_for_plan(e, p, c, &dense));
     e->last_count_dense = dense != nullptr;
     PC_TRY(count_prepare(e, p, dense != nullptr));
@@ -3045,14 +3109,18 @@
     return count_finish(e, p, c);
 }
 
+int64_t pc_dense_set_cells(pc_engine *e) {
+    if (!e || e->files.empty() || e->knobs.no_dense || !e->last_count_dense) return -1;
+    const DenseVector &dv = e->dvec;
+    return (dv.dsig_valid && dv.dsig == dense_sig(e)) ? dv.dcells : -1;
+}
+
 int64_t pc_dense_cells(pc_engine *e, int file) {
-    if (!e || file < 0 || file >= (int)e->files.size()) return -1;
-    const StagedFile *sf = e->files[file];
-    if (e->files.size() != 1 || e->knobs.no_dense || !e->last_count_dense) return -1;
-    return (sf->dsig_valid && sf->dsig == dense_sig(e, sf)) ? sf->dcells : -1;
-}
-
-int pc_dense_path(pc_engine *e) { return e && pc_dense_cells(e, 0) >= 0 ? e->last_dense_path : PC_DENSE_PATH_NONE; }
+    if (!e || file < 0 || file >= (int)e->files.size() || e->files.size() != 1) return -1;
+    return pc_dense_set_cells(e);
+}
+
+int pc_dense_path(pc_engine *e) { return pc_dense_set_cells(e) >= 0 ? e->last_dense_path : PC_DENSE_PATH_NONE; }
 
 int pc_sync(pc_engine *e) {
     if (!e) return fail(PC_ERR_ARG, "engine is NULL");
diff --git a/plastid_amd/engine.py b/plastid_amd/engine.py
--- a/plastid_amd/engine.py
+++ b/plastid_amd/engine.py
@@ -160,6 +160,9 @@
     def dense_cells(self, file_index):
         return int(self._lib.pc_dense_cells(self._h, int(file_index)))
 
+    def dense_set_cells(self):
+        return int(self._lib.pc_dense_set_cells(self._h))
+
     def dense_path(self):
         return {1: "items", 2: "chunks"}.get(int(self._lib.pc_dense_path(self._h)))
 
```

After: 2102 billion reads/s (median of 3 runs). Within noise of the previous version (-0.0%).
